# kallenordling/cesm_emulator

Hardware: NVIDIA B200
Metric: train samples/s (baseline cfg) (higher is better)
Workload: dtype fp16

## Files before the change

### cesm_emulator_b200/_lib.py

```python
from __future__ import annotations

import ctypes
from ctypes import POINTER, Structure, c_char_p, c_float, c_int32, c_int64, c_void_p
from pathlib import Path

_PKG = Path(__file__).resolve().parent
LIB_PATH = _PKG / "libcesm_b200.so"

CESM_MAX_TAPS = 16


class IgemmArgs(Structure):

    _fields_ = [
        ("a0", c_void_p), ("a1", c_void_p),
        ("c0", c_int32), ("c1", c_int32),
        ("n", c_int32), ("h", c_int32), ("w", c_int32),
        ("stride", c_int32),
        ("num_taps", c_int32),
        ("tap_dh", c_int32 * CESM_MAX_TAPS), ("tap_dw", c_int32 * CESM_MAX_TAPS),
        ("wt", c_void_p), ("cout", c_int32),
        ("oh", c_int32), ("ow", c_int32),
        ("out", c_void_p), ("ldo", c_int32),
        ("out_h", c_int32), ("out_w", c_int32),
        ("o_sh", c_int32), ("o_sw", c_int32), ("o_h0", c_int32), ("o_w0", c_int32),
        ("bias", c_void_p), ("residual", c_void_p), ("ldr", c_int32),
        ("gn_sums", c_void_p), ("gn_groups", c_int32), ("gn_frames", c_int32),
        ("ln_colsum", c_void_p), ("ln_eps", ctypes.c_float), ("reserved_", c_int32),
    ]


class WgradArgs(Structure):

    _fields_ = [
        ("x0", c_void_p), ("x1", c_void_p),
        ("c0", c_int32), ("c1", c_int32),
        ("n", c_int32), ("h", c_int32), ("w", c_int32),
        ("stride", c_int32),
        ("num_taps", c_int32),
        ("tap_dh", c_int32 * CESM_MAX_TAPS), ("tap_dw", c_int32 * CESM_MAX_TAPS),
        ("dy", c_void_p), ("cout", c_int32),
        ("oh", c_int32), ("ow", c_int32),
        ("y_h", c_int32), ("y_w", c_int32),
        ("y_sh", c_int32), ("y_sw", c_int32), ("y_h0", c_int32), ("y_w0", c_int32),
        ("dw", c_void_p),
        ("dw_so", ctypes.c_longlong), ("dw_si", ctypes.c_longlong),
        ("dw_tap_off", c_int32 * CESM_MAX_TAPS),
    ]


class PackDesc(Structure):

    _fields_ = [
        ("src", c_void_p), ("dst", c_void_p),
        ("O", c_int32), ("T", c_int32), ("I", c_int32), ("pad_", c_int32),
        ("so", ctypes.c_longlong), ("si", ctypes.c_longlong),
        ("tap_off", c_int32 * CESM_MAX_TAPS),
    ]


class FilmDesc(Structure):

    _fields_ = [("W", c_void_p), ("bias", c_void_p), ("dW", c_void_p), ("db", c_void_p), ("N", c_int32), ("n0", c_int32)]


class CesmError(RuntimeError):
    pass


_lib = None


def load() -> ctypes.CDLL:
    global _lib
    if _lib is not None:
        return _lib
    if not LIB_PATH.exists():
        raise CesmError(
            f"{LIB_PATH} not found: build it with `python -m cesm_emulator_b200.build` "
            "(there is no CPU or PyTorch fallback for the B200 kernels)")
    lib = ctypes.CDLL(str(LIB_PATH))
    lib.cesm_last_error.restype = c_char_p
    lib.cesm_version.restype = c_char_p
    lib.cesm_launch_count.restype = ctypes.c_longlong
    lib.cesm_linattn_ws_floats.restype = ctypes.c_size_t
    lib.cesm_linattn_ws_floats.argtypes = [ctypes.c_int, ctypes.c_int]
    lib.cesm_adamw_partials.restype = ctypes.c_int
    lib.cesm_tattn_long_max_frames.restype = ctypes.c_int
    lib.cesm_set_prezeroed_scratch.restype = None
    lib.cesm_set_prezeroed_scratch.argtypes = [ctypes.c_int]
    _declare(lib)
    _lib = lib
    return lib


_P, _I, _L, _F = c_void_p, ctypes.c_int, ctypes.c_longlong, c_float
_SIGNATURES: dict[str, list] = {
    "cesm_igemm": [POINTER(IgemmArgs), _P],
    "cesm_wgrad": [POINTER(WgradArgs), _P],
    "cesm_pack_weight": [_P, _P, _I, _I, _I, _L, _L, POINTER(c_int32), _P],
    "cesm_pack_weights_batched": [_P, _I, _P],
    "cesm_unpack_wgrads_batched": [_P, _I, _P],
    "cesm_unpack_wgrad": [_P, _P, _I, _I, _I, _L, _L, POINTER(c_int32), _I, _P],
    "cesm_adamw_step": [_P, _P, _P, _P, _L, _P, _P, _F, _F, _F, _F, _P],
    "cesm_adamw_ema_step": [_P, _P, _P, _P, _P, _L, _P, _P, _F, _F, _F, _F, ctypes.c_double, _L, _P],
    "cesm_colsum": [_P, _P, _L, _I, _I, _P],
    "cesm_gn_stats": [_P, _P, _I, _L, _I, _I, _P],
    "cesm_gn_apply_fwd": [_P, _P, _P, _P, _P, _P, _P, _I, _L, _I, _I, _F, _P],
    "cesm_gn_bwd": [_P, _P, _P, _P, _P, _P, _P, _P, _P, _P, _P, _P, _I, _L, _I, _I, _F, _I, _P],
    "cesm_ln_fwd": [_P, _P, _P, _L, _I, _F, _P],
    "cesm_ln_bwd": [_P, _P, _P, _P, _P, _P, _L, _I, _F, _I, _P],
    "cesm_tattn_fwd": [_P, _P, _P, _P, _P, _P, _I, _I, _I, _I, _I, _F, _P],
    "cesm_tattn_bwd": [_P, _P, _P, _P, _P, _P, _P, _P, _P, _I, _I, _I, _I, _I, _F, _P],
    "cesm_tattn_proj_fwd": [_P, _P, _P, _P, _P, _P, _I, _I, _I, _I, _I, _I, _F, _P],
    "cesm_tattn_long_fwd": [_P, _P, _P, _P, _P, _P, _I, _I, _I, _I, _I, _F, _P],
    "cesm_tattn_long_bwd": [_P, _P, _P, _P, _P, _P, _P, _P, _P, _I, _I, _I, _I, _I, _F, _P],
    "cesm_mattn_fwd": [_P, _P, _P, _I, _I, _I, _I, _F, _P],
    "cesm_mattn_bwd": [_P, _P, _P, _P, _P, _P, _I, _I, _I, _I, _F, _P],
    "cesm_linattn_fwd": [_P, _P, _P, _I, _I, _I, _I, _F, _P],
    "cesm_linattn_bwd": [_P, _P, _P, _P, _P, _I, _I, _I, _I, _F, _P],
    "cesm_film_fwd": [_P, _P, _P, _I, _I, _I, _I, _P],
    "cesm_film_bwd": [_P, _P, _P, _I, _I, _P, _I, _I, _I, _P],
    "cesm_gather_windows": [_P, _P, _P, _P, _P, _I, _I, _I, _I, _I, _I, _I, _I, _P],
    "cesm_qkv_bwd": [_P, _P, _P, _P, _P, _L, _L, _I, _I, _P],
    "cesm_input_patches": [_P, _P, _I, _I, _P, _I, _I, _I, _I, _I, _I, _P],
    "cesm_input_weight_pack": [_P, _P, _P, _I, _I, _I, _P],
    "cesm_input_conv_fwd": [_P, _P, _I, _I, _P, _P, _P, _I, _I, _I, _I, _I, _I, _P],
    "cesm_input_conv_wgrad": [_P, _P, _I, _I, _P, _P, _P, _I, _I, _I, _I, _I, _I, _P],
    "cesm_out_conv_fwd": [_P, _P, _P, _P, _I, _I, _I, _L, _I, _P],
    "cesm_out_conv_bwd": [_P, _P, _P, _P, _P, _P, _I, _I, _I, _L, _I, _P],
    "cesm_sinusoidal": [_P, _P, _I, _I, _P],
    "cesm_small_linear_fwd": [_P, _P, _P, _P, _I, _I, _I, _I, _P],
    "cesm_small_linear_bwd": [_P, _P, _P, _P, _P, _P, _I, _I, _I, _I, _I, _P],
    "cesm_q_sample": [_P, _P, _P, _P, _P, _P, _I, _L, _P],
    "cesm_mse_fwd": [_P, _P, _P, _P, _L, _P],
    "cesm_scale_by_scalar": [_P, _P, _F, _P, _L, _P],
    "cesm_p_sample": [_P, _P, _P, _P, _P, _P, _P, _P, _P, _I, _L, _P],
    "cesm_ddim_step": [_P, _P, _P, _P, _P, _P, _P, _P, _I, _I, _L, _P],
    "cesm_dpm_step": [_P, _P, _P, _P, _P, _P, _P, _P, _I, _I, _L, _P],
}


def _declare(lib: ctypes.CDLL) -> None:
    for name, argtypes in _SIGNATURES.items():
        fn = getattr(lib, name)
        fn.argtypes = argtypes
        fn.restype = ctypes.c_int


def exported_symbols() -> list[str]:
    return ["cesm_last_error", "cesm_version", "cesm_launch_count", "cesm_linattn_ws_floats", "cesm_adamw_partials",
            "cesm_set_prezeroed_scratch", "cesm_tattn_long_max_frames",
            *sorted(_SIGNATURES)]


def launch_count() -> int:
    return int(load().cesm_launch_count())


def check(rc: int, what: str) -> None:
    if rc != 0:
        msg = load().cesm_last_error().decode("utf-8", "replace")
        raise CesmError(f"{what} failed (status {rc}): {msg}")


class KernelProfiler:

    def __init__(self):
        self.records = []

    def summary(self):
        import torch
        torch.cuda.synchronize()
        out = {}
        for name, meta, e0, e1 in self.records:
            key = name if not meta or "kind" not in meta else f"{name}/{meta['kind']}"
            d = out.setdefault(key, {"calls": 0, "ms": 0.0, "flops": 0.0, "bytes": 0.0})
            d["calls"] += 1
            d["ms"] += e0.elapsed_time(e1)
            if meta:
                d["flops"] += meta.get("flops", 0.0)
                d["bytes"] += meta.get("bytes", 0.0)
        return out


PROFILER = None
NVTX = bool(int(__import__("os").environ.get("CESM_NVTX", "0")))


def _nvtx_call(lib, name, args, meta):
    from torch.cuda import nvtx
    nvtx.range_push(name if not meta or "kind" not in meta else f"{name}/{meta['kind']}")
    try:
        check(getattr(lib, name)(*args), name)
    finally:
        nvtx.range_pop()


def call(name: str, *args, _meta=None) -> None:
    lib = load()
    prof = PROFILER
    if prof is None:
        if NVTX:
            _nvtx_call(lib, name, args, _meta)
            return
        check(getattr(lib, name)(*args), name)
        return
    import torch
    e0, e1 = torch.cuda.Event(enable_timing=True), torch.cuda.Event(enable_timing=True)
    e0.record()
    check(getattr(lib, name)(*args), name)
    e1.record()
    prof.records.append((name, _meta, e0, e1))
```

### cesm_emulator_b200/csrc/linattn.cu

```cuda
#include "api_common.h"
#include "common.cuh"

namespace cesm {

static constexpr int LD = 32;
static constexpr int SPITCH = 40;

__device__ __forceinline__ void ldmatrix_x4_trans(uint32_t (&r)[4], uint32_t addr) {
    asm volatile("ldmatrix.sync.aligned.m8n8.x4.trans.shared.b16 {%0, %1, %2, %3}, [%4];"
                 : "=r"(r[0]), "=r"(r[1]), "=r"(r[2]), "=r"(r[3])
                 : "r"(addr));
}
__device__ __forceinline__ void mma_16816(float (&c)[4], const uint32_t (&a)[4], uint32_t b0, uint32_t b1) {
    asm volatile(
        "mma.sync.aligned.m16n8k16.row.col.f32.f16.f16.f32 {%0, %1, %2, %3}, {%4, %5, %6, %7}, {%8, %9}, "
        "{%0, %1, %2, %3};"
        : "+f"(c[0]), "+f"(c[1]), "+f"(c[2]), "+f"(c[3])
        : "r"(a[0]), "r"(a[1]), "r"(a[2]), "r"(a[3]), "r"(b0), "r"(b1));
}
__device__ __forceinline__ uint32_t enc_ordered(float f) {
    const uint32_t b = __float_as_uint(f);
    return (b & 0x80000000u) ? ~b : (b | 0x80000000u);
}
__device__ __forceinline__ float dec_ordered(uint32_t u) {
    return __uint_as_float((u & 0x80000000u) ? (u & 0x7fffffffu) : ~u);
}
__device__ __forceinline__ void unpack8(const uint4& u, float (&f)[8]) {
    float2 a = unpack_h2(u.x), b = unpack_h2(u.y), c = unpack_h2(u.z), d = unpack_h2(u.w);
    f[0] = a.x; f[1] = a.y; f[2] = b.x; f[3] = b.y; f[4] = c.x; f[5] = c.y; f[6] = d.x; f[7] = d.y;
}
__device__ __forceinline__ uint4 pack8(const float (&f)[8]) {
    uint4 u;
    u.x = pack_h2(f[0], f[1]); u.y = pack_h2(f[2], f[3]);
    u.z = pack_h2(f[4], f[5]); u.w = pack_h2(f[6], f[7]);
    return u;
}
__device__ __forceinline__ float quad_max(float v) {
    v = fmaxf(v, __shfl_xor_sync(0xffffffffu, v, 1));
    return fmaxf(v, __shfl_xor_sync(0xffffffffu, v, 2));
}
__device__ __forceinline__ float quad_sum(float v) {
    v += __shfl_xor_sync(0xffffffffu, v, 1);
    return v + __shfl_xor_sync(0xffffffffu, v, 2);
}

__device__ __forceinline__ void cp_async16(uint32_t dst, const void* src) {
    asm volatile("cp.async.cg.shared.global [%0], [%1], 16;" ::"r"(dst), "l"(src) : "memory");
}
__device__ __forceinline__ void cp_async_commit() { asm volatile("cp.async.commit_group;" ::: "memory"); }
template <int N>
__device__ __forceinline__ void cp_async_wait() {
    asm volatile("cp.async.wait_group %0;" ::"n"(N) : "memory");
}
static constexpr int kTileBytes = 16 * SPITCH * 2;

struct LaWs {
    uint32_t* kmax;
    float* z;
    float* ctx;
};
__device__ __forceinline__ LaWs la_ws(float* ws, int ni, int HD, int H) {
    float* base = ws + (size_t)ni * (2 * HD + (size_t)H * LD * LD);
    return {reinterpret_cast<uint32_t*>(base), base + HD, base + 2 * HD};
}

__global__ void __launch_bounds__(256)
la_colmax_kernel(const h16* __restrict__ qkv, float* __restrict__ ws, int n, int H, int rows_per_block) {
    pdl_trigger();
    pdl_wait();
    const int HD = H * LD, cpr = HD / 8;
    const int ni = blockIdx.y;
    const int chunk = threadIdx.x % cpr, rl = threadIdx.x / cpr, nrl = blockDim.x / cpr;
    const int p0 = blockIdx.x * rows_per_block, p1 = min(n, p0 + rows_per_block);
    float m[8];
#pragma unroll
    for (int i = 0; i < 8; ++i) m[i] = -INFINITY;
    if (rl < nrl) {
        const h16* base = qkv + ((size_t)ni * n) * (3 * HD) + HD + chunk * 8;
        for (int p = p0 + rl; p < p1; p += nrl) {
            float f[8];
            unpack8(__ldg(reinterpret_cast<const uint4*>(base + (size_t)p * 3 * HD)), f);
#pragma unroll
            for (int i = 0; i < 8; ++i) m[i] = fmaxf(m[i], f[i]);
        }
    }
    __shared__ float red[256][9];
#pragma unroll
    for (int i = 0; i < 8; ++i) red[threadIdx.x][i] = m[i];
    __syncthreads();
    if ((int)threadIdx.x < HD) {
        const int c = threadIdx.x, ch = c / 8, i = c % 8;
        float v = -INFINITY;
        for (int r = 0; r < nrl; ++r) v = fmaxf(v, red[r * cpr + ch][i]);
        if (v > -INFINITY) atomicMax(la_ws(ws, ni, HD, H).kmax + c, enc_ordered(v));
    }
}

static constexpr int CTX_STAGES = 3;
template <int MODE>
__global__ void __launch_bounds__(256)
la_context_kernel(const h16* __restrict__ qkv, const h16* __restrict__ dout,
                  float* __restrict__ ws, float* __restrict__ acc_out , int n, int H,
                  int chunk, float scale) {
    pdl_trigger();
    pdl_wait();
    extern __shared__ __align__(16) uint8_t la_smem[];
    const int HD = H * LD, ld = 3 * HD;
    const int ni = blockIdx.y, w = threadIdx.x >> 5, lane = threadIdx.x & 31;
    const int r = lane >> 2, c = lane & 3;
    constexpr int kWarpTiles = 2 * CTX_STAGES + (MODE == 1 ? 1 : 0);
    uint8_t* wbase = la_smem + (size_t)w * kWarpTiles * kTileBytes;
    h16* sA = reinterpret_cast<h16*>(wbase + 2 * CTX_STAGES * kTileBytes);
    const uint32_t sA_addr = smem_u32(sA);
    const uint32_t ring_addr = smem_u32(wbase);
    const LaWs W = la_ws(ws, ni, HD, H);

    float cmf[2][2], zf[2][2];
#pragma unroll
    for (int mt = 0; mt < 2; ++mt)
#pragma unroll
        for (int hh = 0; hh < 2; ++hh) {
            cmf[mt][hh] = (MODE == 0) ? dec_ordered(W.kmax[w * LD + 16 * mt + r + 8 * hh]) * kLog2e : 0.f;
            zf[mt][hh] = 0.f;
        }
    float acc[2][4][4];
#pragma unroll
    for (int a = 0; a < 2; ++a)
#pragma unroll
        for (int b = 0; b < 4; ++b)
#pragma unroll
            for (int k = 0; k < 4; ++k) acc[a][b][k] = 0.f;

    const size_t img_row0 = (size_t)ni * n;
    const h16* a_base = qkv + img_row0 * ld + (MODE == 0 ? HD : 0) + w * LD + c * 8;
    const h16* b_base = (MODE == 0) ? qkv + img_row0 * ld + 2 * HD + w * LD + c * 8
                                              : dout + img_row0 * HD + w * LD + c * 8;
    const int b_ld = (MODE == 0) ? ld : HD;
    const int p0 = blockIdx.x * chunk, p1 = min(n, p0 + chunk);

    const int mi = lane >> 3, rr = lane & 7;
    uint32_t a_off[2], b_off[2];
#pragma unroll
    for (int mt = 0; mt < 2; ++mt) a_off[mt] = (((mi >> 1) * 8 + rr) * SPITCH + 16 * mt + (mi & 1) * 8) * 2;
#pragma unroll
    for (int jp = 0; jp < 2; ++jp) b_off[jp] = (((mi & 1) * 8 + rr) * SPITCH + 8 * (jp * 2 + (mi >> 1))) * 2;

    auto issue_loads = [&](int step) {
        const int pp = p0 + 16 * step;
        const uint32_t st = ring_addr + (step % CTX_STAGES) * 2 * kTileBytes;
        if (pp < p1) {
#pragma unroll
            for (int h2 = 0; h2 < 2; ++h2) {
                const int row = min(pp + r + 8 * h2, p1 - 1);
                const uint32_t off = ((r + 8 * h2) * SPITCH + c * 8) * 2;
                cp_async16(st + off, a_base + (size_t)row * ld);
                cp_async16(st + kTileBytes + off, b_base + (size_t)row * b_ld);
            }
        }
        cp_async_commit();
    };
    const int nsteps = (p1 - p0 + 15) / 16;
#pragma unroll
    for (int s0 = 0; s0 < CTX_STAGES - 1; ++s0) issue_loads(s0);
    for (int step = 0; step < nsteps; ++step) {
        const int p = p0 + 16 * step;
        issue_loads(step + CTX_STAGES - 1);
        cp_async_wait<CTX_STAGES - 1>();
        __syncwarp();
        const uint32_t st = ring_addr + (step % CTX_STAGES) * 2 * kTileBytes;
        const uint32_t sB_addr = st + kTileBytes;
        uint32_t af[2][4], bf[2][4];
        if (MODE == 0) {
            ldmatrix_x4_trans(af[0], st + a_off[0]);
            ldmatrix_x4_trans(af[1], st + a_off[1]);
            const bool full = p + 16 <= p1;
#pragma unroll
            for (int mt = 0; mt < 2; ++mt)
#pragma unroll
                for (int i = 0; i < 4; ++i) {
                    const float2 x = unpack_h2(af[mt][i]);
                    float e0 = exp_sub(x.x, cmf[mt][i & 1]), e1 = exp_sub(x.y, cmf[mt][i & 1]);
                    if (!full) {
                        const int px = p + 2 * c + 8 * (i >> 1);
                        e0 = px < p1 ? e0 : 0.f;
                        e1 = px + 1 < p1 ? e1 : 0.f;
                    }
                    zf[mt][i & 1] += e0 + e1;
                    af[mt][i] = pack_h2(e0, e1);
                }
        } else {
            uint4 ua[2];
#pragma unroll
            for (int h2 = 0; h2 < 2; ++h2) {
                const uint32_t off = ((r + 8 * h2) * SPITCH + c * 8) * 2;
                asm volatile("ld.shared.v4.b32 {%0, %1, %2, %3}, [%4];"
                             : "=r"(ua[h2].x), "=r"(ua[h2].y), "=r"(ua[h2].z), "=r"(ua[h2].w)
                             : "r"(st + off));
            }
#pragma unroll
            for (int h2 = 0; h2 < 2; ++h2) {
                const bool valid = (p + r + 8 * h2) < p1;
                float f[8];
                unpack8(ua[h2], f);
                float m = f[0];
#pragma unroll
                for (int i = 1; i < 8; ++i) m = fmaxf(m, f[i]);
                m = quad_max(m) * kLog2e;
                float sum = 0.f;
#pragma unroll
                for (int i = 0; i < 8; ++i) {
                    f[i] = exp_sub(f[i], m);
                    sum += f[i];
                }
                sum = quad_sum(sum);
                const float inv = valid ? scale / sum : 0.f;
#pragma unroll
                for (int i = 0; i < 8; ++i) f[i] *= inv;
                *reinterpret_cast<uint4*>(sA + (r + 8 * h2) * SPITCH + c * 8) = pack8(f);
            }
            __syncwarp();
            ldmatrix_x4_trans(af[0], sA_addr + a_off[0]);
            ldmatrix_x4_trans(af[1], sA_addr + a_off[1]);
        }
        ldmatrix_x4_trans(bf[0], sB_addr + b_off[0]);
        ldmatrix_x4_trans(bf[1], sB_addr + b_off[1]);
        __syncwarp();
#pragma unroll
        for (int mt = 0; mt < 2; ++mt)
#pragma unroll
            for (int j = 0; j < 4; ++j) mma_16816(acc[mt][j], af[mt], bf[j >> 1][(j & 1) * 2], bf[j >> 1][(j & 1) * 2 + 1]);
    }

    float* dst = (MODE == 0 ? W.ctx : acc_out + (size_t)ni * H * LD * LD) + (size_t)w * LD * LD;
    const int g = lane >> 2, t = lane & 3;
#pragma unroll
    for (int mt = 0; mt < 2; ++mt)
#pragma unroll
        for (int j = 0; j < 4; ++j) {
            const int d0 = 16 * mt + g, e0 = 8 * j + 2 * t;
            atomicAdd(dst + d0 * LD + e0, acc[mt][j][0]);
            atomicAdd(dst + d0 * LD + e0 + 1, acc[mt][j][1]);
            atomicAdd(dst + (d0 + 8) * LD + e0, acc[mt][j][2]);
            atomicAdd(dst + (d0 + 8) * LD + e0 + 1, acc[mt][j][3]);
        }
    if (MODE == 0) {
#pragma unroll
        for (int mt = 0; mt < 2; ++mt)
#pragma unroll
            for (int hh = 0; hh < 2; ++hh) {
                const float z = quad_sum(zf[mt][hh]);
                if (c == 0) atomicAdd(W.z + w * LD + 16 * mt + r + 8 * hh, z);
            }
    }
}

__global__ void la_finalize_kernel(float* __restrict__ ws, int H, int NI) {
    pdl_trigger();
    pdl_wait();
    const int HD = H * LD;
    const int idx = blockIdx.x * blockDim.x + threadIdx.x;
    const int per = H * LD * LD;
    if (idx >= NI * per) return;
    const int ni = idx / per, x = idx % per;
    const LaWs W = la_ws(ws, ni, HD, H);
    W.ctx[x] = W.ctx[x] / W.z[x / LD];
}

__global__ void la_delta_kernel(float* __restrict__ ws, const float* __restrict__ dctx, float* __restrict__ delta,
                                int H, int NI) {
    pdl_trigger();
    pdl_wait();
    const int HD = H * LD;
    const int idx = blockIdx.x * blockDim.x + threadIdx.x;
    if (idx >= NI * HD) return;
    const int ni = idx / HD, hd = idx % HD;
    const LaWs W = la_ws(ws, ni, HD, H);
    const float* dc = dctx + ((size_t)ni * HD + hd) * LD;
    float s = 0.f;
#pragma unroll
    for (int e = 0; e < LD; ++e) s = fmaf(W.ctx[hd * LD + e], dc[e], s);
    delta[idx] = s;
}

__device__ __forceinline__ int phi32(int L) { return ((L >> 1) & 3) * 8 + (L >> 3) * 2 + (L & 1); }

template <bool TRANS>
__device__ __forceinline__ void load_bfrag32(const float* __restrict__ M, int g, int t, uint32_t (&b)[2][4][2]) {
#pragma unroll
    for (int ks = 0; ks < 2; ++ks)
#pragma unroll
        for (int j = 0; j < 4; ++j) {
            const int nn = phi32(8 * j + g);
#pragma unroll
            for (int hi = 0; hi < 2; ++hi) {
                const int k0 = phi32(16 * ks + 8 * hi + 2 * t), k1 = k0 + 1;
                b[ks][j][hi] = TRANS ? pack_h2(M[nn * LD + k0], M[nn * LD + k1])
                                     : pack_h2(M[k0 * LD + nn], M[k1 * LD + nn]);
            }
        }
}
__device__ __forceinline__ void rows_to_afrag(const uint4& lo, const uint4& hi, uint32_t (&a)[2][4]) {
    a[0][0] = lo.x; a[0][1] = hi.x; a[0][2] = lo.y; a[0][3] = hi.y;
    a[1][0] = lo.z; a[1][1] = hi.z; a[1][2] = lo.w; a[1][3] = hi.w;
}
__device__ __forceinline__ void frag_gemm(const uint32_t (&a)[2][4], const uint32_t (&b)[2][4][2], float (&c)[4][4]) {
#pragma unroll
    for (int j = 0; j < 4; ++j) {
        c[j][0] = c[j][1] = c[j][2] = c[j][3] = 0.f;
#pragma unroll
        for (int ks = 0; ks < 2; ++ks) mma_16816(c[j], a[ks], b[ks][j][0], b[ks][j][1]);
    }
}
__device__ __forceinline__ void c_to_rows(const float (&c)[4][4], float (&o)[2][8]) {
#pragma unroll
    for (int j = 0; j < 4; ++j) {
        o[0][2 * j] = c[j][0]; o[0][2 * j + 1] = c[j][1];
        o[1][2 * j] = c[j][2]; o[1][2 * j + 1] = c[j][3];
    }
}
__device__ __forceinline__ void row_softmax(float (&f)[8]) {
    float m = f[0];
#pragma unroll
    for (int i = 1; i < 8; ++i) m = fmaxf(m, f[i]);
    m = quad_max(m) * kLog2e;
    float s = 0.f;
#pragma unroll
    for (int i = 0; i < 8; ++i) {
        f[i] = exp_sub(f[i], m);
        s += f[i];
    }
    const float inv = 1.f / quad_sum(s);
#pragma unroll
    for (int i = 0; i < 8; ++i) f[i] *= inv;
}

static constexpr int APPLY_MT = 2;
static constexpr int RING_STAGES = 3;
__device__ __forceinline__ uint4 lds16(uint32_t addr) {
    uint4 u;
    asm volatile("ld.shared.v4.b32 {%0, %1, %2, %3}, [%4];" : "=r"(u.x), "=r"(u.y), "=r"(u.z), "=r"(u.w) : "r"(addr));
    return u;
}
__global__ void __launch_bounds__(256, 3)
la_apply_kernel(const h16* __restrict__ qkv, float* __restrict__ ws, h16* __restrict__ out, int n,
                int H, int chunk, float scale) {
    pdl_trigger();
    pdl_wait();
    extern __shared__ __align__(16) uint8_t la_smem[];
    const int HD = H * LD, ld = 3 * HD;
    const int ni = blockIdx.y, w = threadIdx.x >> 5, lane = threadIdx.x & 31;
    const int r = lane >> 2, c = lane & 3;
    const LaWs W = la_ws(ws, ni, HD, H);
    uint32_t bctx[2][4][2];
    load_bfrag32<false>(W.ctx + (size_t)w * LD * LD, r, c, bctx);
    const size_t row0 = (size_t)ni * n;
    const int p1 = min(n, (int)(blockIdx.x + 1) * chunk);
    const h16* qbase = qkv + row0 * ld + w * LD + c * 8;
    h16* obase = out + row0 * HD + w * LD + c * 8;
    const uint32_t ring = smem_u32(la_smem) + threadIdx.x * 16u;
    constexpr uint32_t kVec = 256 * 16, kStage = APPLY_MT * 2 * kVec;
    auto issue_loads = [&](int pp, int stage) {
        if (pp < p1) {
#pragma unroll
            for (int mt = 0; mt < APPLY_MT; ++mt)
#pragma unroll
                for (int h2 = 0; h2 < 2; ++h2) {
                    const int row = min(pp + 16 * mt + r + 8 * h2, p1 - 1);
                    cp_async16(ring + stage * kStage + (mt * 2 + h2) * kVec, qbase + (size_t)row * ld);
                }
        }
        cp_async_commit();
    };
    const int pstart = blockIdx.x * chunk;
#pragma unroll
    for (int s0 = 0; s0 < RING_STAGES - 1; ++s0) issue_loads(pstart + s0 * 16 * APPLY_MT, s0);
    int stage = 0;
    for (int p = pstart; p < p1; p += 16 * APPLY_MT) {
        {
            int ns = stage + RING_STAGES - 1;
            if (ns >= RING_STAGES) ns -= RING_STAGES;
            issue_loads(p + (RING_STAGES - 1) * 16 * APPLY_MT, ns);
        }
        cp_async_wait<RING_STAGES - 1>();
        uint4 cq[APPLY_MT][2];
#pragma unroll
        for (int mt = 0; mt < APPLY_MT; ++mt)
#pragma unroll
            for (int h2 = 0; h2 < 2; ++h2) cq[mt][h2] = lds16(ring + stage * kStage + (mt * 2 + h2) * kVec);
        if (++stage == RING_STAGES) stage = 0;
#pragma unroll
        for (int mt = 0; mt < APPLY_MT; ++mt) {
            uint4 pk[2];
#pragma unroll
            for (int h2 = 0; h2 < 2; ++h2) {
                float f[8];
                unpack8(cq[mt][h2], f);
                row_softmax(f);
#pragma unroll
                for (int i = 0; i < 8; ++i) f[i] *= scale;
                pk[h2] = pack8(f);
            }
            uint32_t a[2][4];
            rows_to_afrag(pk[0], pk[1], a);
            float cfr[4][4], o[2][8];
            frag_gemm(a, bctx, cfr);
            c_to_rows(cfr, o);
#pragma unroll
            for (int h2 = 0; h2 < 2; ++h2) {
                const int row = p + 16 * mt + r + 8 * h2;
                if (row < p1) *reinterpret_cast<uint4*>(obase + (size_t)row * HD) = pack8(o[h2]);
            }
        }
    }
}

__global__ void __launch_bounds__(256, 2)
la_bwd_apply_kernel(const h16* __restrict__ qkv, const h16* __restrict__ dout,
                    float* __restrict__ ws, const float* __restrict__ dctx, const float* __restrict__ delta,
                    h16* __restrict__ dqkv, int n, int H, int chunk, float scale) {
    pdl_trigger();
    pdl_wait();
    extern __shared__ __align__(16) uint8_t la_smem[];
    const int HD = H * LD, ld = 3 * HD;
    const int ni = blockIdx.y, w = threadIdx.x >> 5, lane = threadIdx.x & 31;
    const int r = lane >> 2, c = lane & 3;
    const LaWs W = la_ws(ws, ni, HD, H);
    const float* dcx = dctx + ((size_t)ni * H + w) * LD * LD;
    uint32_t b_ctxT[2][4][2], b_dctxT[2][4][2], b_dctx[2][4][2];
    load_bfrag32<true>(W.ctx + (size_t)w * LD * LD, r, c, b_ctxT);
    load_bfrag32<true>(dcx, r, c, b_dctxT);
    load_bfrag32<false>(dcx, r, c, b_dctx);
    __shared__ __align__(16) float s_kml[8 * LD], s_del[8 * LD];
    {
        const int col = threadIdx.x;
        s_kml[col] = (dec_ordered(W.kmax[col]) + __logf(W.z[col])) * kLog2e;
        s_del[col] = delta[(size_t)ni * HD + col];
    }
    __syncthreads();
    const float* kml = s_kml + w * LD + c * 8;
    const float* del = s_del + w * LD + c * 8;
    const size_t row0 = (size_t)ni * n;
    const int p1 = min(n, (int)(blockIdx.x + 1) * chunk);
    const h16* xbase = qkv + row0 * ld + w * LD + c * 8;
    const h16* dbase = dout + row0 * HD + w * LD + c * 8;
    h16* gbase = dqkv + row0 * ld + w * LD + c * 8;
    const uint32_t ring = smem_u32(la_smem) + threadIdx.x * 16u;
    constexpr uint32_t kVec = 256 * 16, kStage = 8 * kVec;
    auto issue_loads = [&](int pp, int stage) {
        if (pp < p1) {
#pragma unroll
            for (int h2 = 0; h2 < 2; ++h2) {
                const int row = min(pp + r + 8 * h2, p1 - 1);
                const h16* xg = xbase + (size_t)row * ld;
                const uint32_t st = ring + stage * kStage + h2 * 4 * kVec;
                cp_async16(st, dbase + (size_t)row * HD);
                cp_async16(st + kVec, xg);
                cp_async16(st + 2 * kVec, xg + HD);
                cp_async16(st + 3 * kVec, xg + 2 * HD);
            }
        }
        cp_async_commit();
    };
    const int pstart = blockIdx.x * chunk;
#pragma unroll
    for (int s0 = 0; s0 < RING_STAGES - 1; ++s0) issue_loads(pstart + s0 * 16, s0);
    int stage = 0;
    for (int p = pstart; p < p1; p += 16) {
        {
            int ns = stage + RING_STAGES - 1;
            if (ns >= RING_STAGES) ns -= RING_STAGES;
            issue_loads(p + (RING_STAGES - 1) * 16, ns);
        }
        cp_async_wait<RING_STAGES - 1>();
        float sm[2][8];
        uint4 ud[2], uv[2], uk[2];
#pragma unroll
        for (int h2 = 0; h2 < 2; ++h2) {
            const uint32_t st = ring + stage * kStage + h2 * 4 * kVec;
            ud[h2] = lds16(st);
            unpack8(lds16(st + kVec), sm[h2]);
            uk[h2] = lds16(st + 2 * kVec);
            uv[h2] = lds16(st + 3 * kVec);
        }
        if (++stage == RING_STAGES) stage = 0;
#pragma unroll
        for (int h2 = 0; h2 < 2; ++h2) row_softmax(sm[h2]);
        uint32_t a[2][4];
        float cfr[4][4], o[2][8];
        rows_to_afrag(ud[0], ud[1], a);
        frag_gemm(a, b_ctxT, cfr);
        c_to_rows(cfr, o);
#pragma unroll
        for (int h2 = 0; h2 < 2; ++h2) {
            float dot = 0.f;
#pragma unroll
            for (int i = 0; i < 8; ++i) dot = fmaf(sm[h2][i], o[h2][i], dot);
            dot = quad_sum(dot);
#pragma unroll
            for (int i = 0; i < 8; ++i) o[h2][i] = sm[h2][i] * scale * (o[h2][i] - dot);
            const int row = p + r + 8 * h2;
            if (row < p1) *reinterpret_cast<uint4*>(gbase + (size_t)row * ld) = pack8(o[h2]);
        }
        rows_to_afrag(uv[0], uv[1], a);
        frag_gemm(a, b_dctxT, cfr);
        c_to_rows(cfr, o);
        uint4 ukh[2];
#pragma unroll
        for (int h2 = 0; h2 < 2; ++h2) {
            float kh[8], km[8], dl[8];
            unpack8(uk[h2], kh);
            *reinterpret_cast<float4*>(km) = *reinterpret_cast<const float4*>(kml);
            *reinterpret_cast<float4*>(km + 4) = *reinterpret_cast<const float4*>(kml + 4);
            *reinterpret_cast<float4*>(dl) = *reinterpret_cast<const float4*>(del);
            *reinterpret_cast<float4*>(dl + 4) = *reinterpret_cast<const float4*>(del + 4);
#pragma unroll
            for (int i = 0; i < 8; ++i) {
                kh[i] = exp_sub(kh[i], km[i]);
                o[h2][i] = kh[i] * (o[h2][i] - dl[i]);
            }
            ukh[h2] = pack8(kh);
            const int row = p + r + 8 * h2;
            if (row < p1) *reinterpret_cast<uint4*>(gbase + (size_t)row * ld + HD) = pack8(o[h2]);
        }
        rows_to_afrag(ukh[0], ukh[1], a);
        frag_gemm(a, b_dctx, cfr);
        c_to_rows(cfr, o);
#pragma unroll
        for (int h2 = 0; h2 < 2; ++h2) {
            const int row = p + r + 8 * h2;
            if (row < p1) *reinterpret_cast<uint4*>(gbase + (size_t)row * ld + 2 * HD) = pack8(o[h2]);
        }
    }
}

}

using namespace cesm;

static int la_chunk(int n, int NI) {
    int chunk = 2048;
    while (chunk > 128 && (long long)NI * ((n + chunk - 1) / chunk) < 148 * 4) chunk >>= 1;
    return chunk;
}

static size_t la_context_smem(int H, int mode) {
    static bool cfg = false;
    if (!cfg) {
        cudaFuncSetAttribute(la_context_kernel<0>, cudaFuncAttributeMaxDynamicSharedMemorySize, 8 * 2 * CTX_STAGES * kTileBytes);
        cudaFuncSetAttribute(la_context_kernel<1>, cudaFuncAttributeMaxDynamicSharedMemorySize, 8 * (2 * CTX_STAGES + 1) * kTileBytes);
        cfg = true;
    }
    return (size_t)H * (2 * CTX_STAGES + (mode == 1 ? 1 : 0)) * kTileBytes;
}

extern "C" size_t cesm_linattn_ws_floats(int NI, int H) { return (size_t)NI * (2 * H * LD + (size_t)H * LD * LD); }

extern "C" int cesm_linattn_fwd(const void* qkv, float* ws, void* out, int NI, int n, int H, int dim_head, float scale,
                                void* stream) {
    CESM_REQUIRE(dim_head == LD, "linear attention kernel needs dim_head == 32 (got %d)", dim_head);
    CESM_REQUIRE(H >= 1 && H <= 8, "linear attention kernel supports 1..8 heads (got %d)", H);
    cudaStream_t st = as_stream(stream);
    const int HD = H * LD;
    CESM_ZERO_SCRATCH(ws, sizeof(float) * cesm_linattn_ws_floats(NI, H), st);
    const int chunk = la_chunk(n, NI);
    dim3 grid(ceil_div(n, chunk), NI);
    launch_pdl(la_colmax_kernel, grid, 256, 0, st, (const h16*)qkv, ws, n, H, chunk);
    CESM_CHECK_LAUNCH();
    const size_t sh = la_context_smem(H, 0);
    launch_pdl(la_context_kernel<0>, grid, 32 * H, sh, st, (const h16*)qkv, nullptr, ws, nullptr, n, H, chunk, scale);
    CESM_CHECK_LAUNCH();
    launch_pdl(la_finalize_kernel, ceil_div(NI * H * LD * LD, 256), 256, 0, st, ws, H, NI);
    CESM_CHECK_LAUNCH();
    const size_t sh_apply = (size_t)RING_STAGES * APPLY_MT * 2 * 256 * 16;
    launch_pdl(la_apply_kernel, grid, 32 * H, sh_apply, st, (const h16*)qkv, ws, (h16*)out, n, H, chunk,
                                                    scale);
    CESM_CHECK_LAUNCH();
    (void)HD;
    return CESM_OK;
}

extern "C" int cesm_linattn_bwd(const void* qkv, float* ws, const void* dout, float* scratch, void* dqkv, int NI, int n,
                                int H, int dim_head, float scale, void* stream) {
    CESM_REQUIRE(dim_head == LD, "linear attention kernel needs dim_head == 32 (got %d)", dim_head);
    CESM_REQUIRE(H >= 1 && H <= 8, "linear attention kernel supports 1..8 heads (got %d)", H);
    cudaStream_t st = as_stream(stream);
    float* dctx = scratch;
    float* delta = scratch + (size_t)NI * H * LD * LD;
    CESM_ZERO_SCRATCH(dctx, sizeof(float) * NI * H * LD * LD, st);
    const int chunk = la_chunk(n, NI);
    dim3 grid(ceil_div(n, chunk), NI);
    const size_t sh = la_context_smem(H, 1);
    launch_pdl(la_context_kernel<1>, grid, 32 * H, sh, st, (const h16*)qkv, (const h16*)dout, ws, dctx, n, H,
                                                   chunk, scale);
    CESM_CHECK_LAUNCH();
    launch_pdl(la_delta_kernel, ceil_div(NI * H * LD, 128), 128, 0, st, ws, dctx, delta, H, NI);
    CESM_CHECK_LAUNCH();
    const size_t sh_bwd = (size_t)RING_STAGES * 8 * 256 * 16;
    static bool bwd_cfg = false;
    if (!bwd_cfg) {
        CESM_CHECK_CUDA(cudaFuncSetAttribute(la_bwd_apply_kernel, cudaFuncAttributeMaxDynamicSharedMemorySize, (int)sh_bwd));
        bwd_cfg = true;
    }
    launch_pdl(la_bwd_apply_kernel, grid, 32 * H, sh_bwd, st, (const h16*)qkv, (const h16*)dout, ws, dctx, delta,
                                                 (h16*)dqkv, n, H, chunk, scale);
    CESM_CHECK_LAUNCH();
    return CESM_OK;
}
```

### cesm_emulator_b200/kernels.py

```python
from __future__ import annotations

import ctypes
from typing import Optional, Sequence, Tuple

import torch

from . import _lib
from ._lib import IgemmArgs

H16 = torch.float16


def _stream() -> ctypes.c_void_p:
    return ctypes.c_void_p(torch.cuda.current_stream().cuda_stream)


def _ptr(t: Optional[torch.Tensor]) -> Optional[int]:
    return None if t is None else t.data_ptr()


def _req_cuda(*ts: Optional[torch.Tensor]) -> None:
    for t in ts:
        if t is not None and not t.is_cuda:
            raise _lib.CesmError("cesm_emulator_b200 kernels need CUDA tensors (no CPU fallback)")
        if t is not None and not t.is_contiguous():
            raise _lib.CesmError("cesm_emulator_b200 kernels need contiguous tensors")


def _bytes_meta(*ts, kind=None):
    if _lib.PROFILER is None:
        return None
    m = {"bytes": float(sum(t.numel() * t.element_size() for t in ts if t is not None))}
    if kind:
        m["kind"] = kind
    return m


TAPS_3x3 = [(dh, dw) for dh in (-1, 0, 1) for dw in (-1, 0, 1)]
TAPS_1x1 = [(0, 0)]


class ZeroArena:

    def __init__(self, device, floats: int = 4 << 20):
        self.buf = torch.zeros(floats, dtype=torch.float32, device=device)
        self.off = 0
        self.high = 0

    def begin(self) -> None:
        global _ARENA
        if self.high:
            self.buf[:self.high].zero_()
        self.off = 0
        _ARENA = self
        _lib.load().cesm_set_prezeroed_scratch(1)

    def end(self) -> None:
        global _ARENA
        _ARENA = None
        _lib.load().cesm_set_prezeroed_scratch(0)

    def take(self, shape) -> torch.Tensor:
        n = 1
        for d in shape:
            n *= int(d)
        start = self.off
        self.off = start + (n + 63) // 64 * 64
        if self.off > self.buf.numel():
            self.off = start
            return torch.zeros(tuple(shape), dtype=torch.float32, device=self.buf.device)
        self.high = max(self.high, self.off)
        return self.buf[start:start + n].view(*shape)


_ARENA: Optional[ZeroArena] = None


def zero_scratch(shape, device) -> torch.Tensor:
    if _ARENA is not None:
        return _ARENA.take(tuple(shape))
    return torch.empty(tuple(shape), dtype=torch.float32, device=device)


def igemm(a0: torch.Tensor, wt: torch.Tensor, *, taps: Sequence[Tuple[int, int]] = TAPS_1x1,
          a1: Optional[torch.Tensor] = None, stride: int = 1,
          out: Optional[torch.Tensor] = None, out_hw: Optional[Tuple[int, int]] = None,
          out_place: Tuple[int, int, int, int] = (1, 1, 0, 0),
          bias: Optional[torch.Tensor] = None, residual: Optional[torch.Tensor] = None,
          gn_sums: Optional[torch.Tensor] = None, gn_frames: int = 1,
          ln_fold: Optional[Tuple[torch.Tensor, float]] = None):
    _req_cuda(a0, a1, wt, out, bias, residual)
    assert a0.dtype == H16 and wt.dtype == H16 and a0.dim() == 4
    n, h, w, c0 = a0.shape
    c1 = 0 if a1 is None else a1.shape[-1]
    cout = wt.shape[0]
    assert wt.shape[1] == len(taps) * (c0 + c1), (wt.shape, len(taps), c0, c1)
    oh, ow = out_hw if out_hw is not None else (h // stride, w // stride)
    o_sh, o_sw, o_h0, o_w0 = out_place
    if out is None:
        assert out_place == (1, 1, 0, 0)
        out = torch.empty((n, oh, ow, cout), dtype=H16, device=a0.device)
    assert out.dtype == H16, out.dtype
    args = IgemmArgs()
    args.a0, args.a1, args.c0, args.c1 = _ptr(a0), _ptr(a1), c0, c1
    args.n, args.h, args.w, args.stride = n, h, w, stride
    args.num_taps = len(taps)
    for i, (dh, dw) in enumerate(taps):
        args.tap_dh[i], args.tap_dw[i] = dh, dw
    args.wt, args.cout = _ptr(wt), cout
    args.oh, args.ow = oh, ow
    args.out, args.ldo = _ptr(out), out.shape[-1]
    args.out_h, args.out_w = out.shape[1], out.shape[2]
    args.o_sh, args.o_sw, args.o_h0, args.o_w0 = o_sh, o_sw, o_h0, o_w0
    args.bias = _ptr(bias)
    args.residual = _ptr(residual)
    args.ldr = 0 if residual is None else residual.shape[-1]
    if gn_sums is not None:
        assert gn_sums.dtype == torch.float32 and gn_sums.dim() == 3 and gn_sums.shape[0] * gn_frames == n
        args.gn_sums, args.gn_groups, args.gn_frames = _ptr(gn_sums), gn_sums.shape[1], gn_frames
    if ln_fold is not None:
        cs, eps = ln_fold
        assert residual is not None and residual.data_ptr() == a0.data_ptr() and c0 == 64 and cout == 64 and a1 is None
        assert cs.dtype == torch.float32 and cs.numel() == cout and cs.is_cuda
        args.ln_colsum, args.ln_eps = _ptr(cs), float(eps)
    if bias is not None:
        assert bias.dtype == torch.float32 and bias.numel() == cout
    if residual is not None:
        assert residual.dtype == H16 and residual.shape[:3] == out.shape[:3]
    meta = None
    if _lib.PROFILER is not None:
        rows = n * oh * ow
        ktot = len(taps) * (c0 + c1)
        meta = {"kind": f"{len(taps)}tap", "flops": 2.0 * rows * cout * ktot,
                "bytes": 2.0 * (rows * (c0 + c1) * stride * stride + rows * cout + cout * ktot)}
    _lib.call("cesm_igemm", ctypes.byref(args), _stream(), _meta=meta)
    return out


def wgrad(x0: torch.Tensor, dy: torch.Tensor, *, taps: Sequence[Tuple[int, int]] = TAPS_1x1,
          x1: Optional[torch.Tensor] = None, stride: int = 1, grid_hw: Optional[Tuple[int, int]] = None,
          dy_place: Tuple[int, int, int, int] = (1, 1, 0, 0), into: Optional[torch.Tensor] = None,
          layout: Optional[Tuple[int, int, Sequence[int]]] = None) -> torch.Tensor:
    _req_cuda(x0, x1, dy)
    assert x0.dtype == H16 and dy.dtype == H16 and x0.dim() == 4 and dy.dim() == 4
    n, h, w, c0 = x0.shape
    c1 = 0 if x1 is None else x1.shape[-1]
    cout = dy.shape[-1]
    oh, ow = grid_hw if grid_hw is not None else (h // stride, w // stride)
    a = _lib.WgradArgs()
    if into is not None:
        assert layout is not None and into.dtype == torch.float32 and into.is_contiguous()
        dw_ = into
        a.dw_so, a.dw_si = int(layout[0]), int(layout[1])
        for i, o in enumerate(layout[2]):
            a.dw_tap_off[i] = int(o)
    else:
        dw_ = torch.empty((cout, len(taps), c0 + c1), dtype=torch.float32, device=x0.device)
    a.x0, a.x1, a.c0, a.c1 = _ptr(x0), _ptr(x1), c0, c1
    a.n, a.h, a.w, a.stride = n, h, w, stride
    a.num_taps = len(taps)
    for i, (dh, dw) in enumerate(taps):
        a.tap_dh[i], a.tap_dw[i] = dh, dw
    a.dy, a.cout, a.oh, a.ow = _ptr(dy), cout, oh, ow
    a.y_h, a.y_w = dy.shape[1], dy.shape[2]
    a.y_sh, a.y_sw, a.y_h0, a.y_w0 = dy_place
    a.dw = _ptr(dw_)
    meta = None
    if _lib.PROFILER is not None:
        rows = n * oh * ow
        meta = {"kind": f"{len(taps)}tap", "flops": 2.0 * rows * cout * len(taps) * (c0 + c1),
                "bytes": 2.0 * rows * (c0 + c1 + cout) + 4.0 * cout * len(taps) * (c0 + c1)}
    _lib.call("cesm_wgrad", ctypes.byref(a), _stream(), _meta=meta)
    return dw_


def qkv_bwd(dy: torch.Tensor, x: torch.Tensor, wt: torch.Tensor, dw_into: Optional[torch.Tensor] = None):
    _req_cuda(dy, x, wt, dw_into)
    assert dy.dtype == H16 and x.dtype == H16 and wt.dtype == H16 and dy.is_contiguous() and x.is_contiguous()
    cout, cin = dy.shape[-1], x.shape[-1]
    rows = x.numel() // cin
    assert dy.numel() // cout == rows and tuple(wt.shape) == (cin, cout) and wt.is_contiguous()
    dx = torch.empty_like(x)
    if dw_into is None:
        dw = torch.zeros((cout, cin), dtype=torch.float32, device=x.device)
    else:
        assert dw_into.dtype == torch.float32 and dw_into.is_contiguous() and dw_into.numel() == cout * cin
        dw = dw_into
    meta = None
    if _lib.PROFILER is not None:
        meta = {"kind": "qkv", "flops": 4.0 * rows * cout * cin, "bytes": 2.0 * rows * (cout + 2 * cin)}
    _lib.call("cesm_qkv_bwd", _ptr(dy), _ptr(x), _ptr(wt), _ptr(dx), _ptr(dw), cin, rows, cin, cout, _stream(), _meta=meta)
    return dx, dw


def _tap_array(offs: Sequence[int]):
    arr = (ctypes.c_int32 * _lib.CESM_MAX_TAPS)()
    for i, o in enumerate(offs):
        arr[i] = int(o)
    return arr


def pack_weight(src: torch.Tensor, O: int, T: int, I: int, so: int, si: int, tap_off: Sequence[int],
                out: Optional[torch.Tensor] = None) -> torch.Tensor:
    _req_cuda(src)
    assert src.dtype == torch.float32
    if out is None:
        out = torch.empty((O, T * I), dtype=H16, device=src.device)
    _lib.call("cesm_pack_weight", _ptr(src), _ptr(out), O, T, I, so, si, _tap_array(tap_off), _stream())
    return out


def unpack_wgrad(src: torch.Tensor, dst: torch.Tensor, O: int, T: int, I: int, so: int, si: int,
                 tap_off: Sequence[int], accumulate: bool = False) -> torch.Tensor:
    _req_cuda(src, dst)
    assert src.dtype == torch.float32 and dst.dtype == torch.float32
    _lib.call("cesm_unpack_wgrad", _ptr(src), _ptr(dst), O, T, I, so, si, _tap_array(tap_off), int(accumulate), _stream())
    return dst


OPT_STATE_FLOATS = 16
OPT_STEP, OPT_NORM, OPT_SCALE, OPT_TRACKER, OPT_FOUND_INF, OPT_SKIPPED, OPT_LR, OPT_WD, OPT_INTERVAL = range(9)


def adamw_step(p: torch.Tensor, g: torch.Tensor, m: torch.Tensor, v: torch.Tensor, partials: torch.Tensor,
               state: torch.Tensor, beta1: float, beta2: float, eps: float, max_norm: Optional[float]) -> None:
    _req_cuda(p, g, m, v, partials, state)
    for t in (p, g, m, v, partials, state):
        assert t.dtype == torch.float32 and t.is_contiguous()
    assert p.numel() == g.numel() == m.numel() == v.numel() and state.numel() >= OPT_STATE_FLOATS
    assert partials.numel() >= _lib.load().cesm_adamw_partials()
    _lib.call("cesm_adamw_step", _ptr(p), _ptr(g), _ptr(m), _ptr(v), p.numel(), _ptr(partials), _ptr(state),
              float(beta1), float(beta2), float(eps), float(max_norm) if max_norm is not None else 0.0, _stream(),
              _meta={"bytes": 28.0 * p.numel()})


def adamw_ema_step(p: torch.Tensor, g: torch.Tensor, m: torch.Tensor, v: torch.Tensor, ema: torch.Tensor,
                   partials: torch.Tensor, state: torch.Tensor, beta1: float, beta2: float, eps: float,
                   max_norm: Optional[float], ema_decay: float, ema_start: int) -> None:
    _req_cuda(p, g, m, v, ema, partials, state)
    for t in (p, g, m, v, ema, partials, state):
        assert t.dtype == torch.float32 and t.is_contiguous()
    assert p.numel() == g.numel() == m.numel() == v.numel() == ema.numel() and state.numel() >= OPT_STATE_FLOATS
    assert partials.numel() >= _lib.load().cesm_adamw_partials()
    _lib.call("cesm_adamw_ema_step", _ptr(p), _ptr(g), _ptr(m), _ptr(v), _ptr(ema), p.numel(), _ptr(partials),
              _ptr(state), float(beta1), float(beta2), float(eps), float(max_norm) if max_norm is not None else 0.0,
              float(ema_decay), int(ema_start), _stream(), _meta={"bytes": 36.0 * p.numel()})


def colsum(x: torch.Tensor, into: Optional[torch.Tensor] = None) -> torch.Tensor:
    _req_cuda(x, into)
    C = x.shape[-1]
    out = torch.empty(C, dtype=torch.float32, device=x.device) if into is None else into
    _lib.call("cesm_colsum", _ptr(x), _ptr(out), x.numel() // C, C, int(into is not None), _stream())
    return out


def gn_stats(x: torch.Tensor, B: int, G: int) -> torch.Tensor:
    _req_cuda(x)
    C = x.shape[-1]
    P = x.numel() // (B * C)
    sums = torch.empty((B, G, 2), dtype=torch.float32, device=x.device)
    _lib.call("cesm_gn_stats", _ptr(x), _ptr(sums), B, P, C, G, _stream(), _meta=_bytes_meta(x))
    return sums


def gn_apply_fwd(x, sums, gamma, beta, film, residual, B: int, G: int, eps: float) -> torch.Tensor:
    _req_cuda(x, sums, gamma, beta, film, residual)
    C = x.shape[-1]
    P = x.numel() // (B * C)
    out = torch.empty_like(x)
    _lib.call("cesm_gn_apply_fwd", _ptr(x), _ptr(sums), _ptr(gamma), _ptr(beta), _ptr(film), _ptr(residual), _ptr(out),
              B, P, C, G, eps, _stream(), _meta=_bytes_meta(x, residual, out))
    return out


def gn_bwd(x, dout, sums, gamma, beta, film, B: int, G: int, eps: float, conv_bias_grad: bool = False,
           into=None):
    _req_cuda(x, dout, sums, gamma, beta, film)
    C = x.shape[-1]
    P = x.numel() // (B * C)
    dev = x.device
    csum = zero_scratch((B, C, 3), dev)
    dx = torch.empty_like(x)
    if into is not None:
        dgamma, dbeta, dcb = into
    else:
        dgamma = torch.empty(C, dtype=torch.float32, device=dev)
        dbeta = torch.empty(C, dtype=torch.float32, device=dev)
        dcb = torch.empty(C, dtype=torch.float32, device=dev) if conv_bias_grad else None
    dfilm = torch.empty((B, 2 * C), dtype=torch.float32, device=dev) if film is not None else None
    _lib.call("cesm_gn_bwd", _ptr(x), _ptr(dout), _ptr(sums), _ptr(gamma), _ptr(beta), _ptr(film), _ptr(csum), _ptr(dx),
              _ptr(dgamma), _ptr(dbeta), _ptr(dfilm), _ptr(dcb), B, P, C, G, eps, int(into is not None), _stream(),
              _meta=_bytes_meta(x, dout, x, dout, dx))
    if conv_bias_grad:
        return dx, dgamma, dbeta, dfilm, dcb
    return dx, dgamma, dbeta, dfilm


def ln_fwd(x: torch.Tensor, gamma: torch.Tensor, eps: float) -> torch.Tensor:
    _req_cuda(x, gamma)
    C = x.shape[-1]
    out = torch.empty_like(x)
    _lib.call("cesm_ln_fwd", _ptr(x), _ptr(gamma), _ptr(out), x.numel() // C, C, eps, _stream(),
              _meta=_bytes_meta(x, out))
    return out


def ln_bwd(x, gamma, dy, dres, eps: float, into: Optional[torch.Tensor] = None):
    _req_cuda(x, gamma, dy, dres, into)
    C = x.shape[-1]
    dx = torch.empty_like(x)
    dgamma = torch.empty(C, dtype=torch.float32, device=x.device) if into is None else into
    _lib.call("cesm_ln_bwd", _ptr(x), _ptr(gamma), _ptr(dy), _ptr(dres), _ptr(dx), _ptr(dgamma), x.numel() // C, C, eps,
              int(into is not None), _stream(), _meta=_bytes_meta(x, dy, dres, dx))
    return dx, dgamma


LONG_WINDOW_MAX = 128


def _bias_to_diag(bias: torch.Tensor) -> torch.Tensor:
    return torch.cat([bias[:, 1:, 0].flip(1), bias[:, 0, :]], dim=1).contiguous()


def _diag_to_bias_grad(ddiag: torch.Tensor, F: int) -> torch.Tensor:
    H = ddiag.shape[0]
    g = torch.zeros((H, F, F), dtype=ddiag.dtype, device=ddiag.device)
    g[:, 0, :] = ddiag[:, F - 1:]
    g[:, 1:, 0] = ddiag[:, :F - 1].flip(1)
    return g


def tattn_fwd(qkv, bias, cs, sn, B: int, F: int, HW: int, H: int, D: int, scale: float):
    _req_cuda(qkv, bias, cs, sn)
    rows = B * F * HW
    out = torch.empty((rows, H * D), dtype=H16, device=qkv.device)
    if 4 < F <= LONG_WINDOW_MAX:
        lse = torch.empty((rows, H), dtype=torch.float32, device=qkv.device)
        _lib.call("cesm_tattn_long_fwd", _ptr(qkv), _ptr(_bias_to_diag(bias)), _ptr(cs), _ptr(sn), _ptr(out), _ptr(lse),
                  B, F, HW, H, D, scale, _stream(),
                  _meta={"kind": f"F{F}", "bytes": float(qkv.numel() * 2 + out.numel() * 2),
                         "flops": 4.0 * rows * H * F * D * 2})
        return out, lse
    lse = torch.empty((rows, H), dtype=torch.float32, device=qkv.device) if F > 4 else None
    _lib.call("cesm_tattn_fwd", _ptr(qkv), _ptr(bias), _ptr(cs), _ptr(sn), _ptr(out), _ptr(lse), B, F, HW, H, D, scale,
              _stream(), _meta=_bytes_meta(qkv, out))
    return out, lse


def tattn_bwd(qkv, bias, cs, sn, out, lse, dout, B: int, F: int, HW: int, H: int, D: int, scale: float):
    _req_cuda(qkv, bias, cs, sn, out, lse, dout)
    dqkv = torch.empty_like(qkv)
    if 4 < F <= LONG_WINDOW_MAX:
        ddiag = zero_scratch((H, 2 * F - 1), qkv.device)
        _lib.call("cesm_tattn_long_bwd", _ptr(qkv), _ptr(_bias_to_diag(bias)), _ptr(cs), _ptr(sn), _ptr(out), _ptr(lse),
                  _ptr(dout), _ptr(dqkv), _ptr(ddiag), B, F, HW, H, D, scale, _stream(),
                  _meta={"kind": f"F{F}", "bytes": float(qkv.numel() * 4 + dout.numel() * 4),
                         "flops": 14.0 * B * F * HW * H * F * D * 2})
        return dqkv, _diag_to_bias_grad(ddiag, F)
    dbias = zero_scratch((H, F, F), qkv.device)
    _lib.call("cesm_tattn_bwd", _ptr(qkv), _ptr(bias), _ptr(cs), _ptr(sn), _ptr(out), _ptr(lse), _ptr(dout), _ptr(dqkv),
              _ptr(dbias), B, F, HW, H, D, scale, _stream(), _meta=_bytes_meta(qkv, dout, dqkv))
    return dqkv, dbias


def tattn_proj_ok(C: int, F: int, HW: int, H: int, D: int) -> bool:
    return C == 64 and 1 <= F <= 3 and HW % 16 == 0 and H == 8 and D == 32


def tattn_proj_fwd(xn, wqkv_packed, bias, cs, sn, B: int, F: int, HW: int, H: int, D: int, scale: float):
    _req_cuda(xn, wqkv_packed, bias, cs, sn)
    assert xn.dtype == H16 and wqkv_packed.dtype == H16 and tuple(wqkv_packed.shape) == (3 * H * D, 64)
    rows = B * F * HW
    out = torch.empty((rows, H * D), dtype=H16, device=xn.device)
    _lib.call("cesm_tattn_proj_fwd", _ptr(xn), _ptr(wqkv_packed), _ptr(bias), _ptr(cs), _ptr(sn), _ptr(out), B, F, HW, H, D,
              64, scale, _stream(),
              _meta={"kind": "fused", "flops": 2.0 * rows * 64 * 3 * H * D, "bytes": float(rows * (64 + H * D) * 2)})
    return out


def mattn_fwd(qkv, NI: int, n: int, H: int, D: int, scale: float):
    _req_cuda(qkv)
    assert qkv.dtype == H16 and qkv.shape == (NI * n, 3 * H * D), (tuple(qkv.shape), NI, n, H, D)
    out = torch.empty((NI * n, H * D), dtype=H16, device=qkv.device)
    lse = torch.empty((NI * n, H), dtype=torch.float32, device=qkv.device)
    _lib.call("cesm_mattn_fwd", _ptr(qkv), _ptr(out), _ptr(lse), NI, n, H, D, scale, _stream(),
              _meta={"kind": "fwd", "flops": 4.0 * NI * H * n * n * D, "bytes": float(qkv.numel() * 2 + out.numel() * 2)})
    return out, lse


def mattn_bwd(qkv, out, lse, dout, NI: int, n: int, H: int, D: int, scale: float):
    _req_cuda(qkv, out, lse, dout)
    assert qkv.dtype == H16 and out.dtype == H16 and dout.dtype == H16 and lse.dtype == torch.float32
    assert qkv.shape == (NI * n, 3 * H * D) and out.shape == dout.shape == (NI * n, H * D) and lse.numel() == NI * n * H
    dqkv = torch.empty_like(qkv)
    delta = torch.empty((NI * n, H), dtype=torch.float32, device=qkv.device)
    _lib.call("cesm_mattn_bwd", _ptr(qkv), _ptr(out), _ptr(lse), _ptr(dout), _ptr(dqkv), _ptr(delta), NI, n, H, D, scale,
              _stream(), _meta={"kind": "bwd", "flops": 14.0 * NI * H * n * n * D,
                                "bytes": float(qkv.numel() * 4 + out.numel() * 2 + dout.numel() * 2)})
    return dqkv


def linattn_fwd(qkv, NI: int, n: int, H: int, D: int, scale: float):
    _req_cuda(qkv)
    dev = qkv.device
    ws = zero_scratch((_lib.load().cesm_linattn_ws_floats(NI, H),), dev)
    out = torch.empty((NI * n, H * D), dtype=H16, device=dev)
    _lib.call("cesm_linattn_fwd", _ptr(qkv), _ptr(ws), _ptr(out), NI, n, H, D, scale, _stream(),
              _meta=_bytes_meta(qkv, out))
    return out, ws


def linattn_bwd(qkv, ws, dout, NI: int, n: int, H: int, D: int, scale: float):
    _req_cuda(qkv, ws, dout)
    scratch = zero_scratch((NI * H * D * D + NI * H * D,), qkv.device)
    dqkv = torch.empty_like(qkv)
    _lib.call("cesm_linattn_bwd", _ptr(qkv), _ptr(ws), _ptr(dout), _ptr(scratch), _ptr(dqkv), NI, n, H, D, scale,
              _stream(), _meta=_bytes_meta(qkv, dout, dqkv))
    return dqkv


def gather_windows(cond, tgt, plan, cond_out, x0_out) -> None:
    _req_cuda(cond, tgt, plan, cond_out, x0_out)
    assert cond.dtype == tgt.dtype == cond_out.dtype == x0_out.dtype == torch.float32 and plan.dtype == torch.int32
    assert cond.is_contiguous() and tgt.is_contiguous() and cond_out.is_contiguous() and x0_out.is_contiguous()
    T, M, H, W = cond.shape
    B, _, K, h, w = cond_out.shape
    assert plan.shape == (B, 6) and plan.is_contiguous() and x0_out.shape == (B, 1, h, w) and tgt.shape == cond.shape
    _lib.call("cesm_gather_windows", _ptr(cond), _ptr(tgt), _ptr(plan), _ptr(cond_out), _ptr(x0_out), B, T, M, H, W, K,
              h, w, _stream())


INPUT_KPAD = 256


def input_patches(in0, in1, B: int, F: int, H: int, W: int, ks: int) -> torch.Tensor:
    _req_cuda(in0, in1)
    f0, f1 = in0.numel() // (B * H * W), in1.numel() // (B * H * W)
    out = torch.empty((B * F, H, W, INPUT_KPAD), dtype=H16, device=in0.device)
    _lib.call("cesm_input_patches", _ptr(in0), _ptr(in1), f0, f1, _ptr(out), B, F, H, W, ks, INPUT_KPAD, _stream(),
              _meta=_bytes_meta(out))
    return out


def input_weight_pack(w, bias, out: Optional[torch.Tensor] = None) -> torch.Tensor:
    _req_cuda(w, bias)
    cout, ks = w.shape[0], w.shape[-1]
    if out is None:
        out = torch.empty((cout, INPUT_KPAD), dtype=H16, device=w.device)
    _lib.call("cesm_input_weight_pack", _ptr(w), _ptr(bias), _ptr(out), cout, ks, INPUT_KPAD, _stream())
    return out


def input_conv_fwd(in0, in1, w, bias, B: int, F: int, H: int, W: int, ks: int):
    _req_cuda(in0, in1, w, bias)
    cout = w.shape[0]
    f0, f1 = in0.numel() // (B * H * W), in1.numel() // (B * H * W)
    out = torch.empty((B * F, H, W, cout), dtype=H16, device=in0.device)
    _lib.call("cesm_input_conv_fwd", _ptr(in0), _ptr(in1), f0, f1, _ptr(w), _ptr(bias), _ptr(out), B, F, H, W, ks, cout,
              _stream())
    return out


def input_conv_wgrad(in0, in1, dy, B: int, F: int, H: int, W: int, ks: int):
    _req_cuda(in0, in1, dy)
    cout = dy.shape[-1]
    f0, f1 = in0.numel() // (B * H * W), in1.numel() // (B * H * W)
    dw = torch.empty((cout, 2, 1, ks, ks), dtype=torch.float32, device=dy.device)
    db = torch.empty(cout, dtype=torch.float32, device=dy.device)
    _lib.call("cesm_input_conv_wgrad", _ptr(in0), _ptr(in1), f0, f1, _ptr(dy), _ptr(dw), _ptr(db), B, F, H, W, ks, cout,
              _stream())
    return dw, db


def out_conv_fwd(a, w, bias, B: int, F: int, H: int, W: int, mid: Optional[int] = None):
    _req_cuda(a, w, bias)
    mid = F // 2 if mid is None else mid
    eps = torch.empty((B, 1, H, W), dtype=torch.float32, device=a.device)
    _lib.call("cesm_out_conv_fwd", _ptr(a), _ptr(w), _ptr(bias), _ptr(eps), B, F, mid, H * W, a.shape[-1], _stream())
    return eps


def out_conv_bwd(a, w, deps, B: int, F: int, H: int, W: int, mid: Optional[int] = None):
    _req_cuda(a, w, deps)
    mid = F // 2 if mid is None else mid
    da = torch.empty_like(a)
    dw = torch.empty_like(w)
    db = torch.empty(1, dtype=torch.float32, device=a.device)
    _lib.call("cesm_out_conv_bwd", _ptr(a), _ptr(w), _ptr(deps), _ptr(da), _ptr(dw), _ptr(db), B, F, mid, H * W,
              a.shape[-1], _stream())
    return da, dw, db


def sinusoidal(t: torch.Tensor, dim: int) -> torch.Tensor:
    _req_cuda(t)
    assert t.dtype == torch.int64
    out = torch.empty((t.numel(), dim), dtype=torch.float32, device=t.device)
    _lib.call("cesm_sinusoidal", _ptr(t), _ptr(out), t.numel(), dim, _stream())
    return out


def small_linear_fwd(x, W, bias, act_silu_in: bool):
    _req_cuda(x, W, bias)
    B, K = x.shape
    N = W.shape[0]
    y = torch.empty((B, N), dtype=torch.float32, device=x.device)
    _lib.call("cesm_small_linear_fwd", _ptr(x), _ptr(W), _ptr(bias), _ptr(y), B, K, N, int(act_silu_in), _stream())
    return y


def small_linear_bwd(x, W, dy, act_silu_in: bool, need_dx: bool, into=None):
    _req_cuda(x, W, dy)
    B, K = x.shape
    N = W.shape[0]
    if into is not None:
        dW, db = into
    else:
        dW = torch.empty_like(W)
        db = torch.empty(N, dtype=torch.float32, device=x.device)
    dx = torch.empty_like(x) if need_dx else None
    _lib.call("cesm_small_linear_bwd", _ptr(x), _ptr(W), _ptr(dy), _ptr(dx), _ptr(dW), _ptr(db), B, K, N,
              int(act_silu_in), int(into is not None), _stream())
    return dx, dW, db


def film_table(Ws, bs, dWs=None, dbs=None) -> torch.Tensor:
    n = len(Ws)
    arr = (_lib.FilmDesc * n)()
    n0 = 0
    for i, d in enumerate(arr):
        d.W, d.bias = Ws[i].data_ptr(), bs[i].data_ptr()
        d.dW = dWs[i].data_ptr() if dWs is not None else 0
        d.db = dbs[i].data_ptr() if dbs is not None else 0
        d.N, d.n0 = Ws[i].shape[0], n0
        n0 += Ws[i].shape[0]
    return torch.frombuffer(bytearray(bytes(arr)), dtype=torch.uint8).to(Ws[0].device)


def film_fwd(x: torch.Tensor, table: torch.Tensor, Ns) -> list:
    _req_cuda(x, table)
    B, K = x.shape
    n_total = int(sum(Ns))
    y = torch.empty(B * n_total, dtype=torch.float32, device=x.device)
    _lib.call("cesm_film_fwd", _ptr(x), _ptr(table), _ptr(y), len(Ns), n_total, B, K, _stream())
    outs, n0 = [], 0
    for N in Ns:
        outs.append(y[B * n0:B * (n0 + N)].view(B, N))
        n0 += N
    return outs


def film_bwd(x: torch.Tensor, table: torch.Tensor, dy_packed: torch.Tensor, Ns, need_dx: bool, accumulate: bool):
    _req_cuda(x, table, dy_packed)
    B, K = x.shape
    n_total = int(sum(Ns))
    assert dy_packed.numel() == B * n_total and dy_packed.dtype == torch.float32 and dy_packed.is_contiguous()
    dx = zero_scratch(x.shape, x.device) if need_dx else None
    _lib.call("cesm_film_bwd", _ptr(x), _ptr(table), _ptr(dy_packed), len(Ns), n_total, _ptr(dx), B, K, int(accumulate),
              _stream())
    return dx


def q_sample(x0, noise, t, sqrt_ac, sqrt_1mac):
    _req_cuda(x0, noise, t, sqrt_ac, sqrt_1mac)
    xt = torch.empty_like(x0)
    B = x0.shape[0]
    _lib.call("cesm_q_sample", _ptr(x0), _ptr(noise), _ptr(t), _ptr(sqrt_ac), _ptr(sqrt_1mac), _ptr(xt), B,
              x0.numel() // B, _stream())
    return xt


def mse_fwd(eps, noise):
    _req_cuda(eps, noise)
    diff = torch.empty_like(eps)
    loss = torch.empty((), dtype=torch.float32, device=eps.device)
    _lib.call("cesm_mse_fwd", _ptr(eps), _ptr(noise), _ptr(diff), _ptr(loss), eps.numel(), _stream())
    return loss, diff


def scale_by_scalar(x, gscale, factor: float):
    _req_cuda(x, gscale)
    out = torch.empty_like(x)
    _lib.call("cesm_scale_by_scalar", _ptr(x), _ptr(gscale), factor, _ptr(out), x.numel(), _stream())
    return out


def p_sample(xt, eps, z, t, betas, sqrt_1mac, sqrt_recip_a, post_var):
    _req_cuda(xt, eps, z, t, betas, sqrt_1mac, sqrt_recip_a, post_var)
    out = torch.empty_like(xt)
    B = xt.shape[0]
    _lib.call("cesm_p_sample", _ptr(xt), _ptr(eps), _ptr(z), _ptr(t), _ptr(betas), _ptr(sqrt_1mac), _ptr(sqrt_recip_a),
              _ptr(post_var), _ptr(out), B, xt.numel() // B, _stream())
    return out


def ddim_step(xt, eps, z, t, coef, T: int, out=None, next_t=None, t_out=None):
    _req_cuda(xt, eps, z, t, coef, out, next_t, t_out)
    assert coef.dtype == torch.float32 and coef.shape == (T, 3), (coef.dtype, tuple(coef.shape), T)
    assert t.dtype == torch.int64 and xt.dtype == eps.dtype == torch.float32 and eps.shape == xt.shape
    assert z is None or (z.dtype == torch.float32 and z.shape == xt.shape)
    assert (t_out is None) == (next_t is None), "next_t and t_out go together"
    assert next_t is None or (next_t.dtype == torch.int64 and next_t.shape == (T,) and t_out.dtype == torch.int64)
    out = torch.empty_like(xt) if out is None else out
    assert out.dtype == torch.float32 and out.shape == xt.shape
    B = xt.shape[0]
    _lib.call("cesm_ddim_step", _ptr(xt), _ptr(eps), _ptr(z), _ptr(t), _ptr(coef), _ptr(next_t), _ptr(t_out), _ptr(out),
              T, B, xt.numel() // B, _stream())
    return out


def dpm_step(xt, eps, hist, t, coef, T: int, out=None, next_t=None, t_out=None):
    _req_cuda(xt, eps, hist, t, coef, out, next_t, t_out)
    assert coef.dtype == torch.float32 and coef.shape == (T, 5), (coef.dtype, tuple(coef.shape), T)
    assert t.dtype == torch.int64 and xt.dtype == eps.dtype == torch.float32 and eps.shape == xt.shape
    assert hist.dtype == torch.float32 and hist.shape == xt.shape
    assert (t_out is None) == (next_t is None), "next_t and t_out go together"
    assert next_t is None or (next_t.dtype == torch.int64 and next_t.shape == (T,) and t_out.dtype == torch.int64)
    out = torch.empty_like(xt) if out is None else out
    assert out.dtype == torch.float32 and out.shape == xt.shape
    B = xt.shape[0]
    _lib.call("cesm_dpm_step", _ptr(xt), _ptr(eps), _ptr(hist), _ptr(t), _ptr(coef), _ptr(next_t), _ptr(t_out),
              _ptr(out), T, B, xt.numel() // B, _stream())
    return out
```

### cesm_emulator_b200/ops.py

```python
from __future__ import annotations

import weakref
from typing import Optional, Tuple

import torch

from . import _lib
from . import kernels as K

H16 = torch.float16

_PHASE_TAPS = {0: [(0, 1), (-1, 3)], 1: [(1, 0), (0, 2)]}


_OUTER_GRAD = [True]


class _Fn(torch.autograd.Function):
    @classmethod
    def apply(cls, *args, **kwargs):
        _OUTER_GRAD[0] = torch.is_grad_enabled()
        return super().apply(*args, **kwargs)


def _train(ctx) -> bool:
    return _OUTER_GRAD[0] and any(ctx.needs_input_grad)


def _c(t: Optional[torch.Tensor]) -> Optional[torch.Tensor]:
    return None if t is None else t.contiguous()


def _phase(ph: int, pw: int):
    taps, koff = [], []
    for dh, kh in _PHASE_TAPS[ph]:
        for dw, kw in _PHASE_TAPS[pw]:
            taps.append((dh, dw))
            koff.append(kh * 4 + kw)
    return taps, koff


_WEIGHT_EPOCH = [0]


def invalidate_weight_cache(*_args, **_kwargs) -> None:
    _WEIGHT_EPOCH[0] += 1


try:
    from torch.optim.optimizer import register_optimizer_step_post_hook as _reg_hook
    _reg_hook(invalidate_weight_cache)
except Exception:
    pass


class _PackEntry:
    __slots__ = ("wref", "src_off", "O", "T", "I", "so", "si", "taps", "out", "key", "serial")


_ENTRIES: list = []
_PLAN = {"n": -1, "ptrs": None, "descs": None}
_PREPACK_SERIAL = [0]


def _key(weight: torch.Tensor):
    return (weight.data_ptr(), weight._version, _WEIGHT_EPOCH[0])


class PackCache:

    def __init__(self):
        self._d = {}

    def get(self, weight: torch.Tensor, tag, spec, train: bool = False) -> torch.Tensor:
        ent = self._d.get(tag)
        if ent is None or ent.wref() is not weight:
            ent = _PackEntry()
            ent.wref = weakref.ref(weight)
            ent.src_off, ent.O, ent.T, ent.I, ent.so, ent.si, ent.taps = spec
            ent.out = torch.empty((ent.O, ent.T * ent.I), dtype=H16, device=weight.device)
            ent.key, ent.serial = None, -1
            self._d[tag] = ent
            _ENTRIES.append(ent)
        key = _key(weight)
        force = (train and weight.is_cuda and torch.cuda.is_current_stream_capturing()
                 and ent.serial != _PREPACK_SERIAL[0])
        if force or ent.key != key:
            src = weight.detach().reshape(-1)
            if ent.src_off:
                src = src[ent.src_off:]
            K.pack_weight(src, ent.O, ent.T, ent.I, ent.so, ent.si, ent.taps, out=ent.out)
            ent.key, ent.serial = key, _PREPACK_SERIAL[0]
        return ent.out

    def __deepcopy__(self, memo):
        return PackCache()


def prepack_all() -> int:
    live = [e for e in _ENTRIES if e.wref() is not None]
    if len(live) != len(_ENTRIES):
        _ENTRIES[:] = live
    if not live:
        return 0
    ptrs = tuple((e.wref().data_ptr(), e.out.data_ptr()) for e in live)
    if _PLAN["n"] != len(live) or _PLAN["ptrs"] != ptrs:
        arr = (_lib.PackDesc * len(live))()
        for d, e in zip(arr, live):
            d.src = e.wref().data_ptr() + 4 * e.src_off
            d.dst = e.out.data_ptr()
            d.O, d.T, d.I, d.so, d.si = e.O, e.T, e.I, e.so, e.si
            for i, o in enumerate(e.taps):
                d.tap_off[i] = int(o)
        host = torch.frombuffer(bytearray(bytes(arr)), dtype=torch.uint8)
        _PLAN.update(n=len(live), ptrs=ptrs, descs=host.to(live[0].out.device))
    _PREPACK_SERIAL[0] += 1
    _lib.call("cesm_pack_weights_batched", _PLAN["descs"].data_ptr(), len(live), K._stream())
    for e in live:
        e.key, e.serial = _key(e.wref()), _PREPACK_SERIAL[0]
    return len(live)


_FOLDS: list = []


def _fold_compute(ent, wqkv, wout, gamma) -> None:
    C, hidden = ent[1].shape[0], ent[4]
    wv = wqkv.detach().reshape(3 * hidden, C)[2 * hidden:].float()
    wo = wout.detach().reshape(C, hidden).float()
    w = wo @ wv
    ent[1].copy_(w)
    if gamma is not None:
        ent[6].copy_(w * gamma.detach().reshape(1, C).float())
        ent[7].copy_(ent[6].float().sum(dim=1))


def _fold_f1(meta, wqkv, wout, hidden: int, C: int, gamma=None):
    key = (_key(wqkv), _key(wout), None if gamma is None else _key(gamma))
    ent = meta.__dict__.get("fold_f1")
    if ent is None or ent[1].device != wqkv.device or (gamma is not None and ent[5] is None):
        dev = wqkv.device
        ent = [None, torch.empty((C, C), dtype=H16, device=dev), weakref.ref(wqkv), weakref.ref(wout), hidden,
               None if gamma is None else weakref.ref(gamma),
               None if gamma is None else torch.empty((C, C), dtype=H16, device=dev),
               None if gamma is None else torch.empty((C,), dtype=torch.float32, device=dev)]
        meta.__dict__["fold_f1"] = ent
        _FOLDS.append(ent)
    if ent[0] != key:
        _fold_compute(ent, wqkv, wout, gamma)
        ent[0] = key
    return ent[1] if gamma is None else (ent[6], ent[7])


def refresh_folds() -> None:
    live = [e for e in _FOLDS if e[2]() is not None and e[3]() is not None and (e[5] is None or e[5]() is not None)]
    _FOLDS[:] = live
    for e in live:
        wqkv, wout = e[2](), e[3]()
        gamma = None if e[5] is None else e[5]()
        key = (_key(wqkv), _key(wout), None if gamma is None else _key(gamma))
        if e[0] != key:
            _fold_compute(e, wqkv, wout, gamma)
            e[0] = key


_GRAD_SINK = [None]


def set_grad_sink(sink) -> None:
    _GRAD_SINK[0] = sink


def _direct(weight: torch.Tensor) -> bool:
    sink = _GRAD_SINK[0]
    return sink is not None and weight.grad is not None and sink.owns(weight)


def _direct_all(*params) -> bool:
    return all(p is not None and _direct(p) for p in params)


def _ready(*params) -> None:
    for p in params:
        _GRAD_SINK[0].ready(p)


_SIDE = [None]
_SIDE_KEEP: list = []


def set_side_stream(stream) -> None:
    _SIDE[0] = stream
    _SIDE_KEEP.clear()


def join_side_stream() -> None:
    side = _SIDE[0]
    if side is not None:
        torch.cuda.current_stream().wait_stream(side)
    _SIDE_KEEP.clear()


class _on_side:

    def __init__(self, *tensors):
        self.side = _SIDE[0] if _GRAD_SINK[0] is not None else None
        self.tensors = tensors
        self.ctx = None

    def __enter__(self):
        if self.side is not None:
            self.side.wait_stream(torch.cuda.current_stream())
            _SIDE_KEEP.append(self.tensors)
            self.ctx = torch.cuda.stream(self.side)
            self.ctx.__enter__()
        return self

    def __exit__(self, *exc):
        if self.ctx is not None:
            self.ctx.__exit__(*exc)
        return False


def _wgrad_into_param(weight, x0, x1, dy, taps, so, si, tap_off, last: bool = True,
                      into: Optional[torch.Tensor] = None, **kw):
    T = len(taps)
    if _direct(weight):
        sink = _GRAD_SINK[0]
        with _on_side(x0, x1, dy):
            if T == 1:
                K.wgrad(x0, dy, x1=x1, taps=taps, into=weight.grad, layout=(so, si, tap_off), **kw)
            else:
                cout = dy.shape[-1]
                ctot = x0.shape[-1] + (0 if x1 is None else x1.shape[-1])
                scratch = sink.scratch(weight, tuple(tap_off), (cout, T, ctot, so, si, list(tap_off)))
                K.wgrad(x0, dy, x1=x1, taps=taps, into=scratch, layout=(T * ctot, 1, [t * ctot for t in range(T)]), **kw)
        if last:
            sink.ready(weight)
        return None
    dwt = torch.zeros_like(weight) if into is None else into
    K.wgrad(x0, dy, x1=x1, taps=taps, into=dwt, layout=(so, si, tap_off), **kw)
    return dwt


def _sq_taps(ks: int):
    r = ks // 2
    return [(kh - r, kw - r) for kh in range(ks) for kw in range(ks)]


def _conv_fwd_weight(cache: PackCache, weight, cout: int, ctot: int, ks: int, train: bool):
    kk = ks * ks
    return cache.get(weight, "fwd", (0, cout, kk, ctot, ctot * kk, kk, list(range(kk))), train)


def _conv_dgrad_weights(cache: PackCache, weight, cout: int, c0: int, c1: int, ks: int, train: bool):
    if not train:
        return None, None
    kk, ctot = ks * ks, c0 + c1
    w0 = cache.get(weight, "dgrad0", (0, c0, kk, cout, kk, ctot * kk, list(range(kk))), train)
    w1 = (cache.get(weight, "dgrad1", (c0 * kk, c1, kk, cout, kk, ctot * kk, list(range(kk))), train)
          if c1 else None)
    return w0, w1


def _bias_grad(bias, dy):
    if bias is not None and _direct_all(bias):
        with _on_side(dy):
            K.colsum(dy, into=bias.grad)
        _ready(bias)
        return None
    return K.colsum(dy)


def _conv_wgrad(weight, x0, x1, dy, ks: int):
    cout = weight.shape[0]
    ctot = x0.shape[-1] + (0 if x1 is None else x1.shape[-1])
    kk = ks * ks
    return _wgrad_into_param(weight, x0, x1, dy, _sq_taps(ks), ctot * kk, kk, list(range(kk)))


class ConvFn(_Fn):

    @staticmethod
    def forward(ctx, x0, x1, weight, bias, residual, ksize: int, cache: PackCache):
        x0, x1, residual = _c(x0), _c(x1), _c(residual)
        cout = weight.shape[0]
        c0 = x0.shape[-1]
        c1 = 0 if x1 is None else x1.shape[-1]
        assert weight.numel() == cout * (c0 + c1) * ksize * ksize, (weight.shape, c0, c1, ksize)
        train = _train(ctx)
        wt = _conv_fwd_weight(cache, weight, cout, c0 + c1, ksize, train)
        ctx.wd = _conv_dgrad_weights(cache, weight, cout, c0, c1, ksize, train)
        y = K.igemm(x0, wt, a1=x1, taps=_sq_taps(ksize), bias=bias, residual=residual)
        ctx.save_for_backward(x0, x1, weight)
        ctx.ksize, ctx.has_bias, ctx.has_res = ksize, bias is not None, residual is not None
        return y

    @staticmethod
    def backward(ctx, dy):
        x0, x1, weight = ctx.saved_tensors
        dy = dy.contiguous()
        ntaps = [(-dh, -dw) for dh, dw in _sq_taps(ctx.ksize)]
        dx0 = dx1 = dwt = db = None
        if ctx.needs_input_grad[0]:
            dx0 = K.igemm(dy, ctx.wd[0], taps=ntaps)
        if x1 is not None and ctx.needs_input_grad[1]:
            dx1 = K.igemm(dy, ctx.wd[1], taps=ntaps)
        if ctx.needs_input_grad[2]:
            dwt = _conv_wgrad(weight, x0, x1, dy, ctx.ksize)
        if ctx.has_bias and ctx.needs_input_grad[3]:
            db = K.colsum(dy)
        dres = dy if (ctx.has_res and ctx.needs_input_grad[4]) else None
        return dx0, dx1, dwt, db, dres, None, None


class DownsampleFn(_Fn):

    TAPS = [(kh - 1, kw - 1) for kh in range(4) for kw in range(4)]

    @staticmethod
    def forward(ctx, x, weight, bias, cache: PackCache):
        x = x.contiguous()
        c = x.shape[-1]
        train = _train(ctx)
        wt = cache.get(weight, "fwd", (0, c, 16, c, c * 16, 16, list(range(16))), train)
        ctx.wd = {(ph, pw): cache.get(weight, ("dgrad", ph, pw), (0, c, 4, c, 16, c * 16, _phase(ph, pw)[1]), train)
                  for ph in (0, 1) for pw in (0, 1)} if train else None
        y = K.igemm(x, wt, taps=DownsampleFn.TAPS, stride=2, bias=bias)
        ctx.save_for_backward(x, weight)
        ctx.bias_ref = bias
        return y

    @staticmethod
    def backward(ctx, dy):
        x, weight = ctx.saved_tensors
        dy = dy.contiguous()
        n, h, w, c = x.shape
        dx = dwt = db = None
        if ctx.needs_input_grad[0]:
            dx = torch.empty_like(x)
            for (ph, pw), wd in ctx.wd.items():
                K.igemm(dy, wd, taps=_phase(ph, pw)[0], out=dx, out_hw=(h // 2, w // 2), out_place=(2, 2, ph, pw))
        if ctx.needs_input_grad[1]:
            dwt = _wgrad_into_param(weight, x, None, dy, DownsampleFn.TAPS, c * 16, 16, list(range(16)), stride=2)
        if ctx.needs_input_grad[2]:
            db = _bias_grad(ctx.bias_ref, dy)
        return dx, dwt, db, None


class UpsampleFn(_Fn):

    @staticmethod
    def forward(ctx, x, weight, bias, cache: PackCache):
        x = x.contiguous()
        n, h, w, c = x.shape
        out = torch.empty((n, 2 * h, 2 * w, c), dtype=H16, device=x.device)
        train = _train(ctx)
        ctx.wd = cache.get(weight, "dgrad", (0, c, 16, c, c * 16, 16, list(range(16))), train) if train else None
        for ph in (0, 1):
            for pw in (0, 1):
                taps, koff = _phase(ph, pw)
                wt = cache.get(weight, ("fwd", ph, pw), (0, c, 4, c, 16, c * 16, koff), train)
                K.igemm(x, wt, taps=taps, out=out, out_hw=(h, w), out_place=(2, 2, ph, pw), bias=bias)
        ctx.save_for_backward(x, weight)
        ctx.bias_ref = bias
        return out

    @staticmethod
    def backward(ctx, dy):
        x, weight = ctx.saved_tensors
        dy = dy.contiguous()
        n, h, w, c = x.shape
        dx = dwt = db = None
        if ctx.needs_input_grad[0]:
            dx = K.igemm(dy, ctx.wd, taps=DownsampleFn.TAPS, stride=2)
        if ctx.needs_input_grad[1]:
            into = None if _direct(weight) else torch.zeros_like(weight)
            for n_ph, (ph, pw) in enumerate([(0, 0), (0, 1), (1, 0), (1, 1)]):
                taps, koff = _phase(ph, pw)
                dwt = _wgrad_into_param(weight, x, None, dy, taps, 16, c * 16, koff, last=(n_ph == 3), into=into,
                                        grid_hw=(h, w), dy_place=(2, 2, ph, pw))
        if ctx.needs_input_grad[2]:
            db = _bias_grad(ctx.bias_ref, dy)
        return dx, dwt, db, None


class GroupNormSiLUFn(_Fn):

    @staticmethod
    def forward(ctx, x, gamma, beta, film, residual, B: int, G: int, eps: float):
        x, film, residual = x.contiguous(), _c(film), _c(residual)
        sums = K.gn_stats(x, B, G)
        out = K.gn_apply_fwd(x, sums, gamma, beta, film, residual, B, G, eps)
        ctx.save_for_backward(x, sums, gamma, beta, film)
        ctx.cfg = (B, G, eps, residual is not None)
        return out

    @staticmethod
    def backward(ctx, dout):
        x, sums, gamma, beta, film = ctx.saved_tensors
        B, G, eps, has_res = ctx.cfg
        dout = dout.contiguous()
        dx, dgamma, dbeta, dfilm = K.gn_bwd(x, dout, sums, gamma, beta, film, B, G, eps)
        return dx, dgamma, dbeta, dfilm, (dout if has_res else None), None, None, None


class LayerNormFn(_Fn):

    @staticmethod
    def forward(ctx, x, gamma, eps: float):
        x = x.contiguous()
        g = gamma.reshape(-1)
        ctx.save_for_backward(x, g)
        ctx.eps, ctx.gshape = eps, gamma.shape
        return K.ln_fwd(x, g, eps)

    @staticmethod
    def backward(ctx, dy):
        x, g = ctx.saved_tensors
        dx, dg = K.ln_bwd(x, g, dy.contiguous(), None, ctx.eps)
        return dx, dg.view(ctx.gshape), None


class TemporalAttnCoreFn(_Fn):

    @staticmethod
    def forward(ctx, qkv, pos_bias, cs, sn, B: int, F: int, HW: int, H: int, D: int):
        qkv, pos_bias = qkv.contiguous(), pos_bias.contiguous().float()
        scale = D ** -0.5
        out, lse = K.tattn_fwd(qkv, pos_bias, cs, sn, B, F, HW, H, D, scale)
        if F <= 4:
            ctx.save_for_backward(qkv, pos_bias, cs, sn)
        else:
            ctx.save_for_backward(qkv, pos_bias, cs, sn, out, lse)
        ctx.dims = (B, F, HW, H, D, scale)
        return out

    @staticmethod
    def backward(ctx, dout):
        B, F, HW, H, D, scale = ctx.dims
        if F <= 4:
            (qkv, pos_bias, cs, sn), out, lse = ctx.saved_tensors, None, None
        else:
            qkv, pos_bias, cs, sn, out, lse = ctx.saved_tensors
        dqkv, dbias = K.tattn_bwd(qkv, pos_bias, cs, sn, out, lse, dout.contiguous(), B, F, HW, H, D, scale)
        return dqkv, dbias, None, None, None, None, None, None, None


class MidAttnCoreFn(_Fn):

    @staticmethod
    def forward(ctx, qkv, NI: int, n: int, H: int, D: int):
        qkv = qkv.contiguous()
        out, lse = K.mattn_fwd(qkv, NI, n, H, D, D ** -0.5)
        ctx.save_for_backward(qkv, out, lse)
        ctx.dims = (NI, n, H, D)
        return out

    @staticmethod
    def backward(ctx, dout):
        qkv, out, lse = ctx.saved_tensors
        NI, n, H, D = ctx.dims
        return K.mattn_bwd(qkv, out, lse, dout.contiguous(), NI, n, H, D, D ** -0.5), None, None, None, None


class RelPosBiasFn(_Fn):

    @staticmethod
    def forward(ctx, weight, idx):
        ctx.save_for_backward(idx)
        ctx.shape = weight.shape
        return weight.detach()[idx].permute(2, 0, 1).float().contiguous()

    @staticmethod
    def backward(ctx, dbias):
        (idx,) = ctx.saved_tensors
        dw = torch.zeros(ctx.shape, dtype=dbias.dtype, device=dbias.device)
        dw.index_add_(0, idx.reshape(-1), dbias.permute(1, 2, 0).reshape(-1, ctx.shape[1]))
        return dw, None


class LinearAttnCoreFn(_Fn):

    @staticmethod
    def forward(ctx, qkv, NI: int, n: int, H: int, D: int):
        qkv = qkv.contiguous()
        scale = D ** -0.5
        out, ws = K.linattn_fwd(qkv, NI, n, H, D, scale)
        ctx.save_for_backward(qkv, ws)
        ctx.dims = (NI, n, H, D, scale)
        return out

    @staticmethod
    def backward(ctx, dout):
        qkv, ws = ctx.saved_tensors
        NI, n, H, D, scale = ctx.dims
        return K.linattn_bwd(qkv, ws, dout.contiguous(), NI, n, H, D, scale), None, None, None, None


class BlockMeta:

    def __init__(self, **kw):
        self.__dict__.update(kw)

    def __deepcopy__(self, memo):
        return BlockMeta(**{k: (PackCache() if isinstance(v, PackCache) else v) for k, v in self.__dict__.items()
                            if k != "fold_f1"})


class ResnetBlockFn(_Fn):

    @staticmethod
    def forward(ctx, x, x1, film, w1, b1, g1w, g1b, w2, b2, g2w, g2b, wres, bres, B, meta):
        x, x1, film = x.contiguous(), _c(x1), _c(film)
        G, eps = meta.G, meta.eps
        c0 = x.shape[-1]
        cx1 = 0 if x1 is None else x1.shape[-1]
        cout = w1.shape[0]
        train = _train(ctx)
        if wres is None:
            res = x
        else:
            res = K.igemm(x, _conv_fwd_weight(meta.cres, wres, cout, c0 + cx1, 1, train), a1=x1, bias=bres)
        F = x.shape[0] // B
        sums1 = K.zero_scratch((B, G, 2), x.device)
        y1 = K.igemm(x, _conv_fwd_weight(meta.c1, w1, cout, c0 + cx1, 3, train), a1=x1, taps=K.TAPS_3x3, bias=b1,
                     gn_sums=sums1, gn_frames=F)
        h1 = K.gn_apply_fwd(y1, sums1, g1w, g1b, film, None, B, G, eps)
        sums2 = K.zero_scratch((B, G, 2), x.device)
        y2 = K.igemm(h1, _conv_fwd_weight(meta.c2, w2, cout, cout, 3, train), taps=K.TAPS_3x3, bias=b2,
                     gn_sums=sums2, gn_frames=F)
        out = K.gn_apply_fwd(y2, sums2, g2w, g2b, None, res, B, G, eps)
        ctx.wd1 = _conv_dgrad_weights(meta.c1, w1, cout, c0, cx1, 3, train)
        ctx.wd2 = _conv_dgrad_weights(meta.c2, w2, cout, cout, 0, 3, train)
        ctx.wdres = None if wres is None else _conv_dgrad_weights(meta.cres, wres, cout, c0, cx1, 1, train)
        ctx.save_for_backward(x, x1, film, y1, sums1, h1, y2, sums2, w1, g1w, g1b, w2, g2w, g2b, wres, b1, b2, bres)
        ctx.cfg = (B, G, eps)
        return out

    @staticmethod
    def backward(ctx, dout):
        x, x1, film, y1, sums1, h1, y2, sums2, w1, g1w, g1b, w2, g2w, g2b, wres, b1, b2, bres = ctx.saved_tensors
        B, G, eps = ctx.cfg
        dout = dout.contiguous()
        ntaps = [(-dh, -dw) for dh, dw in K.TAPS_3x3]
        if _direct_all(g2w, g2b, b2):
            dy2, _, _, _, _ = K.gn_bwd(y2, dout, sums2, g2w, g2b, None, B, G, eps, conv_bias_grad=True,
                                       into=(g2w.grad, g2b.grad, b2.grad))
            _ready(g2w, g2b, b2)
            dg2w = dg2b = db2 = None
        else:
            dy2, dg2w, dg2b, _, db2 = K.gn_bwd(y2, dout, sums2, g2w, g2b, None, B, G, eps, conv_bias_grad=True)
        dw2 = _conv_wgrad(w2, h1, None, dy2, 3)
        dh1 = K.igemm(dy2, ctx.wd2[0], taps=ntaps)
        if _direct_all(g1w, g1b, b1):
            dy1, _, _, dfilm, _ = K.gn_bwd(y1, dh1, sums1, g1w, g1b, film, B, G, eps, conv_bias_grad=True,
                                           into=(g1w.grad, g1b.grad, b1.grad))
            _ready(g1w, g1b, b1)
            dg1w = dg1b = db1 = None
        else:
            dy1, dg1w, dg1b, dfilm, db1 = K.gn_bwd(y1, dh1, sums1, g1w, g1b, film, B, G, eps, conv_bias_grad=True)
        dw1 = _conv_wgrad(w1, x, x1, dy1, 3)
        dx = dx1 = dwres = dbres = None
        if wres is None:
            if ctx.needs_input_grad[0]:
                dx = K.igemm(dy1, ctx.wd1[0], taps=ntaps, residual=dout)
        else:
            if ctx.needs_input_grad[0]:
                r0 = K.igemm(dout, ctx.wdres[0])
                dx = K.igemm(dy1, ctx.wd1[0], taps=ntaps, residual=r0)
            if x1 is not None and ctx.needs_input_grad[1]:
                r1 = K.igemm(dout, ctx.wdres[1])
                dx1 = K.igemm(dy1, ctx.wd1[1], taps=ntaps, residual=r1)
            dwres = _conv_wgrad(wres, x, x1, dout, 1)
            if _direct_all(bres):
                with _on_side(dout):
                    K.colsum(dout, into=bres.grad)
                _ready(bres)
            else:
                dbres = K.colsum(dout)
        return dx, dx1, dfilm, dw1, db1, dg1w, dg1b, dw2, db2, dg2w, dg2b, dwres, dbres, None, None


def _qkv_backward(wqkv, wdq, xn, dqkv4):
    C, cout = xn.shape[-1], dqkv4.shape[-1]
    if C == 64 and cout % 128 == 0 and cout <= 768:
        if _direct(wqkv):
            dxn, _ = K.qkv_bwd(dqkv4, xn, wdq, dw_into=wqkv.grad)
            _ready(wqkv)
            return dxn, None
        dxn, dw = K.qkv_bwd(dqkv4, xn, wdq)
        return dxn, dw.view_as(wqkv)
    return K.igemm(dqkv4, wdq), _conv_wgrad(wqkv, xn, None, dqkv4, 1)


class TemporalAttnBlockFn(_Fn):

    @staticmethod
    def forward(ctx, x, gamma, wqkv, wout, pos_bias, cs, sn, B, F, meta):
        x = x.contiguous()
        NI, H_, W_, C = x.shape
        heads, D, eps = meta.heads, meta.dim_head, meta.eps
        hidden = heads * D
        g = gamma.reshape(-1)
        pos_bias = pos_bias.contiguous().float()
        train = _train(ctx)
        if F == 1 and not train and C == 64:
            wln, colsum = _fold_f1(meta, wqkv, wout, hidden, C, gamma=gamma)
            return K.igemm(x, wln, residual=x, ln_fold=(colsum, eps))
        xn = K.ln_fwd(x, g, eps)
        if F == 1 and not train:
            return K.igemm(xn, _fold_f1(meta, wqkv, wout, hidden, C), residual=x)
        wq = _conv_fwd_weight(meta.cq, wqkv, 3 * hidden, C, 1, train)
        if not train and K.tattn_proj_ok(C, F, H_ * W_, heads, D):
            o = K.tattn_proj_fwd(xn.view(-1, C), wq, pos_bias, cs, sn, B, F, H_ * W_, heads, D, D ** -0.5)
            return K.igemm(o.view(NI, H_, W_, hidden), _conv_fwd_weight(meta.co, wout, C, hidden, 1, train), residual=x)
        qkv = K.igemm(xn, wq)
        o, lse = K.tattn_fwd(qkv.view(-1, 3 * hidden), pos_bias, cs, sn, B, F, H_ * W_, heads, D, D ** -0.5)
        y = K.igemm(o.view(NI, H_, W_, hidden), _conv_fwd_weight(meta.co, wout, C, hidden, 1, train), residual=x)
        ctx.wdq = _conv_dgrad_weights(meta.cq, wqkv, 3 * hidden, C, 0, 1, train)[0]
        ctx.wdo = _conv_dgrad_weights(meta.co, wout, C, hidden, 0, 1, train)[0]
        saved = [x, g, xn, o, pos_bias, cs, sn, wqkv, wout, gamma, qkv]
        if F > 4:
            saved.append(lse)
        ctx.save_for_backward(*saved)
        ctx.cfg, ctx.gshape = (B, F, heads, D, eps), gamma.shape
        return y

    @staticmethod
    def backward(ctx, dy):
        saved = ctx.saved_tensors
        x, g, xn, o, pos_bias, cs, sn, wqkv, wout, gamma, qkv = saved[:11]
        lse = saved[11] if len(saved) > 11 else None
        B, F, heads, D, eps = ctx.cfg
        hidden = heads * D
        NI, H_, W_, C = x.shape
        dy = dy.contiguous()
        do = K.igemm(dy, ctx.wdo)
        dwout = _conv_wgrad(wout, o.view(NI, H_, W_, hidden), None, dy, 1)
        dqkv, dbias = K.tattn_bwd(qkv.view(-1, 3 * hidden), pos_bias, cs, sn, o if F > 4 else None, lse,
                                  do.view(-1, hidden), B, F, H_ * W_, heads, D, D ** -0.5)
        dqkv4 = dqkv.view(NI, H_, W_, 3 * hidden)
        dxn, dwqkv = _qkv_backward(wqkv, ctx.wdq, xn, dqkv4)
        if _direct_all(gamma):
            dx, _ = K.ln_bwd(x, g, dxn, dy, eps, into=gamma.grad.view(-1))
            _ready(gamma)
            dgamma = None
        else:
            dx, dg = K.ln_bwd(x, g, dxn, dy, eps)
            dgamma = dg.view(ctx.gshape)
        return dx, dgamma, dwqkv, dwout, dbias, None, None, None, None, None


class MidAttnBlockFn(_Fn):

    @staticmethod
    def forward(ctx, x, gamma, wqkv, wout, meta):
        x = x.contiguous()
        NI, H_, W_, C = x.shape
        heads, D, eps = meta.heads, meta.dim_head, meta.eps
        hidden, n = heads * D, H_ * W_
        g = gamma.reshape(-1)
        train = _train(ctx)
        xn = K.ln_fwd(x, g, eps)
        qkv = K.igemm(xn, _conv_fwd_weight(meta.cq, wqkv, 3 * hidden, C, 1, train))
        o, lse = K.mattn_fwd(qkv.view(-1, 3 * hidden), NI, n, heads, D, D ** -0.5)
        y = K.igemm(o.view(NI, H_, W_, hidden), _conv_fwd_weight(meta.co, wout, C, hidden, 1, train), residual=x)
        if train:
            ctx.wdq = _conv_dgrad_weights(meta.cq, wqkv, 3 * hidden, C, 0, 1, train)[0]
            ctx.wdo = _conv_dgrad_weights(meta.co, wout, C, hidden, 0, 1, train)[0]
            ctx.save_for_backward(x, g, xn, qkv, o, lse, wqkv, wout, gamma)
            ctx.cfg, ctx.gshape = (heads, D, eps), gamma.shape
        return y

    @staticmethod
    def backward(ctx, dy):
        x, g, xn, qkv, o, lse, wqkv, wout, gamma = ctx.saved_tensors
        heads, D, eps = ctx.cfg
        hidden = heads * D
        NI, H_, W_, C = x.shape
        dy = dy.contiguous()
        do = K.igemm(dy, ctx.wdo)
        dwout = _conv_wgrad(wout, o.view(NI, H_, W_, hidden), None, dy, 1)
        dqkv = K.mattn_bwd(qkv.view(-1, 3 * hidden), o.view(-1, hidden), lse, do.view(-1, hidden), NI, H_ * W_, heads, D,
                           D ** -0.5)
        dxn, dwqkv = _qkv_backward(wqkv, ctx.wdq, xn, dqkv.view(NI, H_, W_, 3 * hidden))
        if _direct_all(gamma):
            dx, _ = K.ln_bwd(x, g, dxn, dy, eps, into=gamma.grad.view(-1))
            _ready(gamma)
            dgamma = None
        else:
            dx, dg = K.ln_bwd(x, g, dxn, dy, eps)
            dgamma = dg.view(ctx.gshape)
        return dx, dgamma, dwqkv, dwout, None


class SpatialAttnBlockFn(_Fn):

    @staticmethod
    def forward(ctx, x, gamma, wqkv, wout, bout, meta):
        x = x.contiguous()
        NI, H_, W_, C = x.shape
        heads, D, eps = meta.heads, meta.dim_head, meta.eps
        hidden = heads * D
        g = gamma.reshape(-1)
        train = _train(ctx)
        xn = K.ln_fwd(x, g, eps)
        qkv = K.igemm(xn, _conv_fwd_weight(meta.cq, wqkv, 3 * hidden, C, 1, train))
        o, ws = K.linattn_fwd(qkv.view(-1, 3 * hidden), NI, H_ * W_, heads, D, D ** -0.5)
        y = K.igemm(o.view(NI, H_, W_, hidden), _conv_fwd_weight(meta.co, wout, C, hidden, 1, train), bias=bout,
                    residual=x)
        ctx.wdq = _conv_dgrad_weights(meta.cq, wqkv, 3 * hidden, C, 0, 1, train)[0]
        ctx.wdo = _conv_dgrad_weights(meta.co, wout, C, hidden, 0, 1, train)[0]
        ctx.save_for_backward(x, g, xn, qkv, o, ws, wqkv, wout, gamma, bout)
        ctx.cfg, ctx.gshape = (heads, D, eps), gamma.shape
        return y

    @staticmethod
    def backward(ctx, dy):
        x, g, xn, qkv, o, ws, wqkv, wout, gamma, bout = ctx.saved_tensors
        heads, D, eps = ctx.cfg
        hidden = heads * D
        NI, H_, W_, C = x.shape
        dy = dy.contiguous()
        do = K.igemm(dy, ctx.wdo)
        dwout = _conv_wgrad(wout, o.view(NI, H_, W_, hidden), None, dy, 1)
        if _direct_all(bout):
            with _on_side(dy):
                K.colsum(dy, into=bout.grad)
            _ready(bout)
            dbout = None
        else:
            dbout = K.colsum(dy)
        dqkv = K.linattn_bwd(qkv.view(-1, 3 * hidden), ws, do.view(-1, hidden), NI, H_ * W_, heads, D, D ** -0.5)
        dqkv4 = dqkv.view(NI, H_, W_, 3 * hidden)
        dxn, dwqkv = _qkv_backward(wqkv, ctx.wdq, xn, dqkv4)
        if _direct_all(gamma):
            dx, _ = K.ln_bwd(x, g, dxn, dy, eps, into=gamma.grad.view(-1))
            _ready(gamma)
            dgamma = None
        else:
            dx, dg = K.ln_bwd(x, g, dxn, dy, eps)
            dgamma = dg.view(ctx.gshape)
        return dx, dgamma, dwqkv, dwout, dbout, None


class InputConvFn(_Fn):

    @staticmethod
    def forward(ctx, x, cond, weight, bias, F: int):
        x, cond = x.contiguous().float(), cond.contiguous().float()
        B, H, W = x.shape[0], x.shape[-2], x.shape[-1]
        ks = weight.shape[-1]
        patches = K.input_patches(x, cond, B, F, H, W, ks)
        out = K.igemm(patches, K.input_weight_pack(weight.detach(), bias.detach()))
        if _train(ctx):
            ctx.save_for_backward(patches, weight, bias)
        return out

    @staticmethod
    def backward(ctx, dy):
        patches, weight, bias = ctx.saved_tensors
        nt = weight[0].numel()
        full = K.wgrad(patches, dy.contiguous())[:, 0, :]
        dw = (full[:, :nt] + full[:, nt:2 * nt]).view_as(weight)
        db = full[:, 2 * nt]
        if _direct_all(weight, bias):
            weight.grad.add_(dw)
            bias.grad.add_(db)
            _ready(weight, bias)
            return None, None, None, None, None
        return None, None, dw, db.contiguous(), None


class OutConvFn(_Fn):

    @staticmethod
    def forward(ctx, a, weight, bias, B: int, F: int, mid: int):
        a = a.contiguous()
        H, W = a.shape[1], a.shape[2]
        ctx.save_for_backward(a, weight)
        ctx.dims = (B, F, H, W, mid)
        return K.out_conv_fwd(a, weight, bias, B, F, H, W, mid)

    @staticmethod
    def backward(ctx, deps):
        a, weight = ctx.saved_tensors
        B, F, H, W, mid = ctx.dims
        da, dw, db = K.out_conv_bwd(a, weight, deps.contiguous().float(), B, F, H, W, mid)
        return da, dw, db, None, None, None


class SmallLinearFn(_Fn):

    @staticmethod
    def forward(ctx, x, weight, bias, act_in: bool):
        x = x.contiguous()
        ctx.save_for_backward(x, weight, bias)
        ctx.act_in = act_in
        return K.small_linear_fwd(x, weight, bias, act_in)

    @staticmethod
    def backward(ctx, dy):
        x, weight, bias = ctx.saved_tensors
        if _direct_all(weight, bias):
            dx, _, _ = K.small_linear_bwd(x, weight, dy.contiguous(), ctx.act_in, ctx.needs_input_grad[0],
                                          into=(weight.grad, bias.grad))
            _ready(weight, bias)
            return dx, None, None, None
        dx, dW, db = K.small_linear_bwd(x, weight, dy.contiguous(), ctx.act_in, ctx.needs_input_grad[0])
        return dx, dW, db, None


_FILM_TABLES: dict = {}


def _film_table(Ws, bs, direct: bool):
    key = (tuple(w.data_ptr() for w in Ws), tuple(b.data_ptr() for b in bs),
           tuple(w.grad.data_ptr() for w in Ws) + tuple(b.grad.data_ptr() for b in bs) if direct else None)
    tab = _FILM_TABLES.get(key)
    if tab is None:
        if len(_FILM_TABLES) > 16:
            _FILM_TABLES.clear()
        tab = K.film_table(Ws, bs, [w.grad for w in Ws], [b.grad for b in bs]) if direct else K.film_table(Ws, bs)
        _FILM_TABLES[key] = tab
    return tab


class FilmAllFn(_Fn):

    @staticmethod
    def forward(ctx, temb, *wb):
        x = temb.contiguous()
        Ws, bs = list(wb[0::2]), list(wb[1::2])
        Ns = [w.shape[0] for w in Ws]
        outs = K.film_fwd(x, _film_table(Ws, bs, False), Ns)
        ctx.save_for_backward(x, *wb)
        ctx.Ns = Ns
        return tuple(outs)

    @staticmethod
    def backward(ctx, *dys):
        x, wb = ctx.saved_tensors[0], ctx.saved_tensors[1:]
        Ws, bs = list(wb[0::2]), list(wb[1::2])
        B = x.shape[0]
        dy = torch.cat([(d if d is not None else x.new_zeros(B, n)).reshape(-1) for d, n in zip(dys, ctx.Ns)])
        if _direct_all(*Ws, *bs):
            dx = K.film_bwd(x, _film_table(Ws, bs, True), dy, ctx.Ns, ctx.needs_input_grad[0], accumulate=True)
            _ready(*Ws, *bs)
            return (dx,) + (None,) * len(wb)
        dWs, dbs = [torch.empty_like(w) for w in Ws], [torch.empty_like(b) for b in bs]
        dx = K.film_bwd(x, K.film_table(Ws, bs, dWs, dbs), dy, ctx.Ns, ctx.needs_input_grad[0], accumulate=False)
        grads = [None] * len(wb)
        grads[0::2], grads[1::2] = dWs, dbs
        return (dx,) + tuple(grads)


class MseLossFn(_Fn):

    @staticmethod
    def forward(ctx, eps, noise):
        loss, diff = K.mse_fwd(eps.contiguous(), noise.contiguous())
        ctx.save_for_backward(diff)
        return loss

    @staticmethod
    def backward(ctx, g):
        (diff,) = ctx.saved_tensors
        g = g.reshape(1).float().contiguous()
        return K.scale_by_scalar(diff, g, 2.0 / diff.numel()), None


def to_cl(x: torch.Tensor) -> Tuple[torch.Tensor, int, int]:
    B, C, F, H, W = x.shape
    return x.permute(0, 2, 3, 4, 1).reshape(B * F, H, W, C).to(H16).contiguous(), B, F


def from_cl(y: torch.Tensor, B: int, F: int) -> torch.Tensor:
    n, H, W, C = y.shape
    return y.view(B, F, H, W, C).permute(0, 4, 1, 2, 3)
```

### include/cesm_b200.h

```cpp
#ifndef CESM_B200_H
#define CESM_B200_H

#include <stddef.h>
#include <stdint.h>

#ifdef __cplusplus
extern "C" {
#endif

typedef enum cesm_status {
    CESM_OK = 0,
    CESM_ERR_INVALID = -1,
    CESM_ERR_CUDA = -2,
    CESM_ERR_INTERNAL = -3
} cesm_status;

const char* cesm_last_error(void);
const char* cesm_version(void);
long long cesm_launch_count(void);


#define CESM_MAX_TAPS 16

typedef struct cesm_igemm_args {
    const void* a0;
    const void* a1;
    int32_t c0, c1;
    int32_t n, h, w;
    int32_t stride;
    int32_t num_taps;
    int32_t tap_dh[CESM_MAX_TAPS];
    int32_t tap_dw[CESM_MAX_TAPS];
    const void* wt;
    int32_t cout;
    int32_t oh, ow;
    void* out;
    int32_t ldo;
    int32_t out_h, out_w, o_sh, o_sw, o_h0, o_w0;
    const float* bias;
    const void* residual;
    int32_t ldr;
    float* gn_sums;
    int32_t gn_groups;
    int32_t gn_frames;
    const float* ln_colsum;
    float ln_eps;
    int32_t reserved_;
} cesm_igemm_args;

int cesm_igemm(const cesm_igemm_args* args, void* stream);

typedef struct cesm_wgrad_args {
    const void* x0;
    const void* x1;
    int32_t c0, c1;
    int32_t n, h, w;
    int32_t stride;
    int32_t num_taps;
    int32_t tap_dh[CESM_MAX_TAPS];
    int32_t tap_dw[CESM_MAX_TAPS];
    const void* dy;
    int32_t cout;
    int32_t oh, ow;
    int32_t y_h, y_w, y_sh, y_sw, y_h0, y_w0;
    float* dw;
    long long dw_so, dw_si;
    int32_t dw_tap_off[CESM_MAX_TAPS];
} cesm_wgrad_args;

int cesm_wgrad(const cesm_wgrad_args* args, void* stream);

int cesm_pack_weight(const float* src, void* dst, int O, int T, int I, long long so, long long si,
                     const int32_t* tap_off, void* stream);
typedef struct cesm_pack_desc {
    const float* src;
    void* dst;
    int32_t O, T, I, pad_;
    long long so, si;
    int32_t tap_off[CESM_MAX_TAPS];
} cesm_pack_desc;
int cesm_pack_weights_batched(const cesm_pack_desc* descs_device, int n, void* stream);
int cesm_unpack_wgrads_batched(const cesm_pack_desc* descs_device, int n, void* stream);
int cesm_qkv_bwd(const void* dy, const void* x, const void* wt, void* dx, float* dw, long long dw_so, long long rows,
                 int cin, int cout, void* stream);

void cesm_set_prezeroed_scratch(int on);

#define CESM_OPT_STATE_FLOATS 16
int cesm_adamw_partials(void);
int cesm_adamw_step(float* p, const float* g, float* m, float* v, long long n, float* partials, float* state,
                    float beta1, float beta2, float eps, float max_norm, void* stream);
int cesm_adamw_ema_step(float* p, const float* g, float* m, float* v, float* ema, long long n, float* partials,
                        float* state, float beta1, float beta2, float eps, float max_norm, double ema_decay,
                        long long ema_start, void* stream);
int cesm_unpack_wgrad(const float* src, float* dst, int O, int T, int I, long long so, long long si,
                      const int32_t* tap_off, int accumulate, void* stream);
int cesm_colsum(const void* x, float* out, long long M, int C, int accumulate, void* stream);

int cesm_gn_stats(const void* x, float* sums, int B, long long P, int C, int G, void* stream);
int cesm_gn_apply_fwd(const void* x, const float* sums, const float* gamma, const float* beta, const float* film,
                      const void* residual, void* out, int B, long long P, int C, int G, float eps, void* stream);
int cesm_gn_bwd(const void* x, const void* dout, const float* sums, const float* gamma, const float* beta,
                const float* film, float* csum, void* dx, float* dgamma, float* dbeta, float* dfilm,
                float* dconv_bias, int B, long long P, int C, int G, float eps, int accumulate_params, void* stream);

int cesm_ln_fwd(const void* x, const float* gamma, void* out, long long M, int C, float eps, void* stream);
int cesm_ln_bwd(const void* x, const float* gamma, const void* dy, const void* dres, void* dx, float* dgamma,
                long long M, int C, float eps, int accumulate, void* stream);

int cesm_tattn_fwd(const void* qkv, const float* bias, const float* cs, const float* sn, void* out, float* lse,
                   int B, int F, int HW, int H, int dim_head, float scale, void* stream);
int cesm_tattn_bwd(const void* qkv, const float* bias, const float* cs, const float* sn, const void* out,
                   const float* lse, const void* dout, void* dqkv, float* dbias, int B, int F, int HW, int H,
                   int dim_head, float scale, void* stream);

int cesm_tattn_proj_fwd(const void* xn, const void* wqkv, const float* bias, const float* cs, const float* sn, void* out,
                        int B, int F, int HW, int H, int dim_head, int cin, float scale, void* stream);

int cesm_tattn_long_max_frames(void);
int cesm_tattn_long_fwd(const void* qkv, const float* bias_diag, const float* cs, const float* sn, void* out,
                        float* lse, int B, int F, int HW, int H, int dim_head, float scale, void* stream);
int cesm_tattn_long_bwd(const void* qkv, const float* bias_diag, const float* cs, const float* sn, const void* out,
                        const float* lse, const void* dout, void* dqkv, float* dbias_diag, int B, int F, int HW, int H,
                        int dim_head, float scale, void* stream);

int cesm_mattn_fwd(const void* qkv, void* out, float* lse, int NI, int n, int H, int dim_head, float scale, void* stream);
int cesm_mattn_bwd(const void* qkv, const void* out, const float* lse, const void* dout, void* dqkv, float* delta, int NI,
                   int n, int H, int dim_head, float scale, void* stream);

size_t cesm_linattn_ws_floats(int NI, int H);
int cesm_linattn_fwd(const void* qkv, float* ws, void* out, int NI, int n, int H, int dim_head, float scale,
                     void* stream);
int cesm_linattn_bwd(const void* qkv, float* ws, const void* dout, float* scratch, void* dqkv, int NI, int n, int H,
                     int dim_head, float scale, void* stream);

typedef struct cesm_film_desc {
    const float* W;
    const float* bias;
    float* dW;
    float* db;
    int32_t N, n0;
} cesm_film_desc;
int cesm_film_fwd(const float* x, const cesm_film_desc* layers_device, float* y, int n_layers, int n_total, int B,
                  int K, void* stream);
int cesm_film_bwd(const float* x, const cesm_film_desc* layers_device, const float* dy, int n_layers, int n_total,
                  float* dx, int B, int K, int accumulate, void* stream);

int cesm_gather_windows(const float* cond, const float* tgt, const int* plan, float* cond_out, float* x0_out, int B,
                        int T, int M, int H, int W, int K, int h, int w, void* stream);

int cesm_input_patches(const float* in0, const float* in1, int f0, int f1, void* out, int B, int F, int H, int W,
                       int ks, int kpad, void* stream);
int cesm_input_weight_pack(const float* w, const float* bias, void* out, int cout, int ks, int kpad, void* stream);
int cesm_input_conv_fwd(const float* in0, const float* in1, int f0, int f1, const float* w, const float* bias,
                        void* out, int B, int F, int H, int W, int ks, int cout, void* stream);
int cesm_input_conv_wgrad(const float* in0, const float* in1, int f0, int f1, const void* dy, float* dw, float* db,
                          int B, int F, int H, int W, int ks, int cout, void* stream);
int cesm_out_conv_fwd(const void* a, const float* w, const float* bias, float* eps, int B, int F, int mid,
                      long long HW, int C, void* stream);
int cesm_out_conv_bwd(const void* a, const float* w, const float* deps, void* da, float* dw, float* db, int B, int F,
                      int mid, long long HW, int C, void* stream);

int cesm_sinusoidal(const long long* t, float* out, int B, int dim, void* stream);
int cesm_small_linear_fwd(const float* x, const float* W, const float* bias, float* y, int B, int K, int N,
                          int act_silu_in, void* stream);
int cesm_small_linear_bwd(const float* x, const float* W, const float* dy, float* dx, float* dW, float* db, int B,
                          int K, int N, int act_silu_in, int accumulate, void* stream);

int cesm_q_sample(const float* x0, const float* noise, const long long* t, const float* sqrt_ac,
                  const float* sqrt_1mac, float* xt, int B, long long per_sample, void* stream);
int cesm_mse_fwd(const float* eps, const float* noise, float* diff, float* loss, long long total, void* stream);
int cesm_scale_by_scalar(const float* in, const float* gscale, float factor, float* out, long long total,
                         void* stream);
int cesm_p_sample(const float* xt, const float* eps, const float* z, const long long* t, const float* betas,
                  const float* sqrt_1mac, const float* sqrt_recip_a, const float* post_var, float* out, int B,
                  long long per_sample, void* stream);
int cesm_ddim_step(const float* xt, const float* eps, const float* z, const long long* t, const float* coef,
                   const long long* next_t, long long* t_out, float* out, int T, int B, long long per_sample,
                   void* stream);
int cesm_dpm_step(const float* xt, const float* eps, float* hist, const long long* t, const float* coef,
                  const long long* next_t, long long* t_out, float* out, int T, int B, long long per_sample,
                  void* stream);

#ifdef __cplusplus
}
#endif
#endif
```

Before: 188.7.

## Fuse linear-attention backward with QKV projection backward in a tcgen05 kernel

Adds a persistent kernel that computes dq/dk/dv rows of the linear-attention backward in registers, stages them in shared memory, and feeds them directly into the QKV projection's dgrad and wgrad GEMMs using TMA, mbarriers and tensor memory. The goal is to avoid writing the dqkv tensor to global memory and reading it back, and to remove the separate GEMM launches. The old per-row math is moved into a shared header so both paths use it. The fused path only runs for C=64, 8 heads of 32, and n a multiple of 128; other shapes fall back to the old path. It adds complex pipeline synchronisation and a weight-gradient accumulation that could limit parallelism.

```diff
diff --git a/cesm_emulator_b200/_lib.py b/cesm_emulator_b200/_lib.py
--- a/cesm_emulator_b200/_lib.py
+++ b/cesm_emulator_b200/_lib.py
@@ -119,6 +119,7 @@
     "cesm_mattn_bwd": [_P, _P, _P, _P, _P, _P, _I, _I, _I, _I, _F, _P],
     "cesm_linattn_fwd": [_P, _P, _P, _I, _I, _I, _I, _F, _P],
     "cesm_linattn_bwd": [_P, _P, _P, _P, _P, _I, _I, _I, _I, _F, _P],
+    "cesm_linattn_qkv_bwd": [_P, _P, _P, _P, _P, _P, _P, _P, _L, _I, _I, _I, _I, _F, _P],
     "cesm_film_fwd": [_P, _P, _P, _I, _I, _I, _I, _P],
     "cesm_film_bwd": [_P, _P, _P, _I, _I, _P, _I, _I, _I, _P],
     "cesm_gather_windows": [_P, _P, _P, _P, _P, _I, _I, _I, _I, _I, _I, _I, _I, _P],
diff --git a/cesm_emulator_b200/csrc/linattn.cu b/cesm_emulator_b200/csrc/linattn.cu
--- a/cesm_emulator_b200/csrc/linattn.cu
+++ b/cesm_emulator_b200/csrc/linattn.cu
@@ -1,9 +1,8 @@
 #include "api_common.h"
-#include "common.cuh"
+#include "linattn_common.cuh"
 
 namespace cesm {
 
-static constexpr int LD = 32;
 static constexpr int SPITCH = 40;
 
 __device__ __forceinline__ void ldmatrix_x4_trans(uint32_t (&r)[4], uint32_t addr) {
@@ -11,38 +10,6 @@
                  : "=r"(r[0]), "=r"(r[1]), "=r"(r[2]), "=r"(r[3])
                  : "r"(addr));
 }
-__device__ __forceinline__ void mma_16816(float (&c)[4], const uint32_t (&a)[4], uint32_t b0, uint32_t b1) {
-    asm volatile(
-        "mma.sync.aligned.m16n8k16.row.col.f32.f16.f16.f32 {%0, %1, %2, %3}, {%4, %5, %6, %7}, {%8, %9}, "
-        "{%0, %1, %2, %3};"
-        : "+f"(c[0]), "+f"(c[1]), "+f"(c[2]), "+f"(c[3])
-        : "r"(a[0]), "r"(a[1]), "r"(a[2]), "r"(a[3]), "r"(b0), "r"(b1));
-}
-__device__ __forceinline__ uint32_t enc_ordered(float f) {
-    const uint32_t b = __float_as_uint(f);
-    return (b & 0x80000000u) ? ~b : (b | 0x80000000u);
-}
-__device__ __forceinline__ float dec_ordered(uint32_t u) {
-    return __uint_as_float((u & 0x80000000u) ? (u & 0x7fffffffu) : ~u);
-}
-__device__ __forceinline__ void unpack8(const uint4& u, float (&f)[8]) {
-    float2 a = unpack_h2(u.x), b = unpack_h2(u.y), c = unpack_h2(u.z), d = unpack_h2(u.w);
-    f[0] = a.x; f[1] = a.y; f[2] = b.x; f[3] = b.y; f[4] = c.x; f[5] = c.y; f[6] = d.x; f[7] = d.y;
-}
-__device__ __forceinline__ uint4 pack8(const float (&f)[8]) {
-    uint4 u;
-    u.x = pack_h2(f[0], f[1]); u.y = pack_h2(f[2], f[3]);
-    u.z = pack_h2(f[4], f[5]); u.w = pack_h2(f[6], f[7]);
-    return u;
-}
-__device__ __forceinline__ float quad_max(float v) {
-    v = fmaxf(v, __shfl_xor_sync(0xffffffffu, v, 1));
-    return fmaxf(v, __shfl_xor_sync(0xffffffffu, v, 2));
-}
-__device__ __forceinline__ float quad_sum(float v) {
-    v += __shfl_xor_sync(0xffffffffu, v, 1);
-    return v + __shfl_xor_sync(0xffffffffu, v, 2);
-}
 
 __device__ __forceinline__ void cp_async16(uint32_t dst, const void* src) {
     asm volatile("cp.async.cg.shared.global [%0], [%1], 16;" ::"r"(dst), "l"(src) : "memory");
@@ -53,16 +20,6 @@
     asm volatile("cp.async.wait_group %0;" ::"n"(N) : "memory");
 }
 static constexpr int kTileBytes = 16 * SPITCH * 2;
-
-struct LaWs {
-    uint32_t* kmax;
-    float* z;
-    float* ctx;
-};
-__device__ __forceinline__ LaWs la_ws(float* ws, int ni, int HD, int H) {
-    float* base = ws + (size_t)ni * (2 * HD + (size_t)H * LD * LD);
-    return {reinterpret_cast<uint32_t*>(base), base + HD, base + 2 * HD};
-}
 
 __global__ void __launch_bounds__(256)
 la_colmax_kernel(const h16* __restrict__ qkv, float* __restrict__ ws, int n, int H, int rows_per_block) {
@@ -280,58 +237,6 @@
 #pragma unroll
     for (int e = 0; e < LD; ++e) s = fmaf(W.ctx[hd * LD + e], dc[e], s);
     delta[idx] = s;
-}
-
-__device__ __forceinline__ int phi32(int L) { return ((L >> 1) & 3) * 8 + (L >> 3) * 2 + (L & 1); }
-
-template <bool TRANS>
-__device__ __forceinline__ void load_bfrag32(const float* __restrict__ M, int g, int t, uint32_t (&b)[2][4][2]) {
-#pragma unroll
-    for (int ks = 0; ks < 2; ++ks)
-#pragma unroll
-        for (int j = 0; j < 4; ++j) {
-            const int nn = phi32(8 * j + g);
-#pragma unroll
-            for (int hi = 0; hi < 2; ++hi) {
-                const int k0 = phi32(16 * ks + 8 * hi + 2 * t), k1 = k0 + 1;
-                b[ks][j][hi] = TRANS ? pack_h2(M[nn * LD + k0], M[nn * LD + k1])
-                                     : pack_h2(M[k0 * LD + nn], M[k1 * LD + nn]);
-            }
-        }
-}
-__device__ __forceinline__ void rows_to_afrag(const uint4& lo, const uint4& hi, uint32_t (&a)[2][4]) {
-    a[0][0] = lo.x; a[0][1] = hi.x; a[0][2] = lo.y; a[0][3] = hi.y;
-    a[1][0] = lo.z; a[1][1] = hi.z; a[1][2] = lo.w; a[1][3] = hi.w;
-}
-__device__ __forceinline__ void frag_gemm(const uint32_t (&a)[2][4], const uint32_t (&b)[2][4][2], float (&c)[4][4]) {
-#pragma unroll
-    for (int j = 0; j < 4; ++j) {
-        c[j][0] = c[j][1] = c[j][2] = c[j][3] = 0.f;
-#pragma unroll
-        for (int ks = 0; ks < 2; ++ks) mma_16816(c[j], a[ks], b[ks][j][0], b[ks][j][1]);
-    }
-}
-__device__ __forceinline__ void c_to_rows(const float (&c)[4][4], float (&o)[2][8]) {
-#pragma unroll
-    for (int j = 0; j < 4; ++j) {
-        o[0][2 * j] = c[j][0]; o[0][2 * j + 1] = c[j][1];
-        o[1][2 * j] = c[j][2]; o[1][2 * j + 1] = c[j][3];
-    }
-}
-__device__ __forceinline__ void row_softmax(float (&f)[8]) {
-    float m = f[0];
-#pragma unroll
-    for (int i = 1; i < 8; ++i) m = fmaxf(m, f[i]);
-    m = quad_max(m) * kLog2e;
-    float s = 0.f;
-#pragma unroll
-    for (int i = 0; i < 8; ++i) {
-        f[i] = exp_sub(f[i], m);
-        s += f[i];
-    }
-    const float inv = 1.f / quad_sum(s);
-#pragma unroll
-    for (int i = 0; i < 8; ++i) f[i] *= inv;
 }
 
 static constexpr int APPLY_MT = 2;
@@ -472,63 +377,35 @@
             issue_loads(p + (RING_STAGES - 1) * 16, ns);
         }
         cp_async_wait<RING_STAGES - 1>();
-        float sm[2][8];
-        uint4 ud[2], uv[2], uk[2];
+        uint4 ud[2], uq[2], uk[2], uv[2];
 #pragma unroll
         for (int h2 = 0; h2 < 2; ++h2) {
             const uint32_t st = ring + stage * kStage + h2 * 4 * kVec;
             ud[h2] = lds16(st);
-            unpack8(lds16(st + kVec), sm[h2]);
+            uq[h2] = lds16(st + kVec);
             uk[h2] = lds16(st + 2 * kVec);
             uv[h2] = lds16(st + 3 * kVec);
         }
         if (++stage == RING_STAGES) stage = 0;
-#pragma unroll
-        for (int h2 = 0; h2 < 2; ++h2) row_softmax(sm[h2]);
-        uint32_t a[2][4];
-        float cfr[4][4], o[2][8];
-        rows_to_afrag(ud[0], ud[1], a);
-        frag_gemm(a, b_ctxT, cfr);
-        c_to_rows(cfr, o);
-#pragma unroll
-        for (int h2 = 0; h2 < 2; ++h2) {
-            float dot = 0.f;
-#pragma unroll
-            for (int i = 0; i < 8; ++i) dot = fmaf(sm[h2][i], o[h2][i], dot);
-            dot = quad_sum(dot);
-#pragma unroll
-            for (int i = 0; i < 8; ++i) o[h2][i] = sm[h2][i] * scale * (o[h2][i] - dot);
-            const int row = p + r + 8 * h2;
-            if (row < p1) *reinterpret_cast<uint4*>(gbase + (size_t)row * ld) = pack8(o[h2]);
-        }
-        rows_to_afrag(uv[0], uv[1], a);
-        frag_gemm(a, b_dctxT, cfr);
-        c_to_rows(cfr, o);
-        uint4 ukh[2];
-#pragma unroll
-        for (int h2 = 0; h2 < 2; ++h2) {
-            float kh[8], km[8], dl[8];
-            unpack8(uk[h2], kh);
-            *reinterpret_cast<float4*>(km) = *reinterpret_cast<const float4*>(kml);
-            *reinterpret_cast<float4*>(km + 4) = *reinterpret_cast<const float4*>(kml + 4);
-            *reinterpret_cast<float4*>(dl) = *reinterpret_cast<const float4*>(del);
-            *reinterpret_cast<float4*>(dl + 4) = *reinterpret_cast<const float4*>(del + 4);
-#pragma unroll
-            for (int i = 0; i < 8; ++i) {
-                kh[i] = exp_sub(kh[i], km[i]);
-                o[h2][i] = kh[i] * (o[h2][i] - dl[i]);
-            }
-            ukh[h2] = pack8(kh);
-            const int row = p + r + 8 * h2;
-            if (row < p1) *reinterpret_cast<uint4*>(gbase + (size_t)row * ld + HD) = pack8(o[h2]);
-        }
-        rows_to_afrag(ukh[0], ukh[1], a);
-        frag_gemm(a, b_dctx, cfr);
-        c_to_rows(cfr, o);
+        uint4 dq[2], dk[2], dv[2];
+        la_bwd_dq_rows(uq, ud, b_ctxT, scale, dq);
 #pragma unroll
         for (int h2 = 0; h2 < 2; ++h2) {
             const int row = p + r + 8 * h2;
-            if (row < p1) *reinterpret_cast<uint4*>(gbase + (size_t)row * ld + 2 * HD) = pack8(o[h2]);
+            if (row < p1) *reinterpret_cast<uint4*>(gbase + (size_t)row * ld) = dq[h2];
+        }
+        uint4 ukh[2];
+        la_bwd_dk_rows(uk, uv, kml, del, b_dctxT, dk, ukh);
+#pragma unroll
+        for (int h2 = 0; h2 < 2; ++h2) {
+            const int row = p + r + 8 * h2;
+            if (row < p1) *reinterpret_cast<uint4*>(gbase + (size_t)row * ld + HD) = dk[h2];
+        }
+        la_bwd_dv_rows(ukh, b_dctx, dv);
+#pragma unroll
+        for (int h2 = 0; h2 < 2; ++h2) {
+            const int row = p + r + 8 * h2;
+            if (row < p1) *reinterpret_cast<uint4*>(gbase + (size_t)row * ld + 2 * HD) = dv[h2];
         }
     }
 }
@@ -579,8 +456,8 @@
     return CESM_OK;
 }
 
-extern "C" int cesm_linattn_bwd(const void* qkv, float* ws, const void* dout, float* scratch, void* dqkv, int NI, int n,
-                                int H, int dim_head, float scale, void* stream) {
+extern "C" int cesm_linattn_bwd_ctx(const void* qkv, float* ws, const void* dout, float* scratch, int NI, int n, int H,
+                                    int dim_head, float scale, void* stream) {
     CESM_REQUIRE(dim_head == LD, "linear attention kernel needs dim_head == 32 (got %d)", dim_head);
     CESM_REQUIRE(H >= 1 && H <= 8, "linear attention kernel supports 1..8 heads (got %d)", H);
     cudaStream_t st = as_stream(stream);
@@ -595,6 +472,18 @@
     CESM_CHECK_LAUNCH();
     launch_pdl(la_delta_kernel, ceil_div(NI * H * LD, 128), 128, 0, st, ws, dctx, delta, H, NI);
     CESM_CHECK_LAUNCH();
+    return CESM_OK;
+}
+
+extern "C" int cesm_linattn_bwd(const void* qkv, float* ws, const void* dout, float* scratch, void* dqkv, int NI, int n,
+                                int H, int dim_head, float scale, void* stream) {
+    const int rc = cesm_linattn_bwd_ctx(qkv, ws, dout, scratch, NI, n, H, dim_head, scale, stream);
+    if (rc) return rc;
+    cudaStream_t st = as_stream(stream);
+    float* dctx = scratch;
+    float* delta = scratch + (size_t)NI * H * LD * LD;
+    const int chunk = la_chunk(n, NI);
+    dim3 grid(ceil_div(n, chunk), NI);
     const size_t sh_bwd = (size_t)RING_STAGES * 8 * 256 * 16;
     static bool bwd_cfg = false;
     if (!bwd_cfg) {
diff --git a/cesm_emulator_b200/csrc/linattn_common.cuh b/cesm_emulator_b200/csrc/linattn_common.cuh
--- /dev/null
+++ b/cesm_emulator_b200/csrc/linattn_common.cuh
@@ -0,0 +1,162 @@
+#pragma once
+#include "common.cuh"
+
+namespace cesm {
+
+static constexpr int LD = 32;
+
+__device__ __forceinline__ void mma_16816(float (&c)[4], const uint32_t (&a)[4], uint32_t b0, uint32_t b1) {
+    asm volatile(
+        "mma.sync.aligned.m16n8k16.row.col.f32.f16.f16.f32 {%0, %1, %2, %3}, {%4, %5, %6, %7}, {%8, %9}, "
+        "{%0, %1, %2, %3};"
+        : "+f"(c[0]), "+f"(c[1]), "+f"(c[2]), "+f"(c[3])
+        : "r"(a[0]), "r"(a[1]), "r"(a[2]), "r"(a[3]), "r"(b0), "r"(b1));
+}
+__device__ __forceinline__ uint32_t enc_ordered(float f) {
+    const uint32_t b = __float_as_uint(f);
+    return (b & 0x80000000u) ? ~b : (b | 0x80000000u);
+}
+__device__ __forceinline__ float dec_ordered(uint32_t u) {
+    return __uint_as_float((u & 0x80000000u) ? (u & 0x7fffffffu) : ~u);
+}
+__device__ __forceinline__ void unpack8(const uint4& u, float (&f)[8]) {
+    float2 a = unpack_h2(u.x), b = unpack_h2(u.y), c = unpack_h2(u.z), d = unpack_h2(u.w);
+    f[0] = a.x; f[1] = a.y; f[2] = b.x; f[3] = b.y; f[4] = c.x; f[5] = c.y; f[6] = d.x; f[7] = d.y;
+}
+__device__ __forceinline__ uint4 pack8(const float (&f)[8]) {
+    uint4 u;
+    u.x = pack_h2(f[0], f[1]); u.y = pack_h2(f[2], f[3]);
+    u.z = pack_h2(f[4], f[5]); u.w = pack_h2(f[6], f[7]);
+    return u;
+}
+__device__ __forceinline__ float quad_max(float v) {
+    v = fmaxf(v, __shfl_xor_sync(0xffffffffu, v, 1));
+    return fmaxf(v, __shfl_xor_sync(0xffffffffu, v, 2));
+}
+__device__ __forceinline__ float quad_sum(float v) {
+    v += __shfl_xor_sync(0xffffffffu, v, 1);
+    return v + __shfl_xor_sync(0xffffffffu, v, 2);
+}
+
+struct LaWs {
+    uint32_t* kmax;
+    float* z;
+    float* ctx;
+};
+__device__ __forceinline__ LaWs la_ws(float* ws, int ni, int HD, int H) {
+    float* base = ws + (size_t)ni * (2 * HD + (size_t)H * LD * LD);
+    return {reinterpret_cast<uint32_t*>(base), base + HD, base + 2 * HD};
+}
+
+__device__ __forceinline__ int phi32(int L) { return ((L >> 1) & 3) * 8 + (L >> 3) * 2 + (L & 1); }
+
+template <bool TRANS>
+__device__ __forceinline__ void load_bfrag32(const float* __restrict__ M, int g, int t, uint32_t (&b)[2][4][2]) {
+#pragma unroll
+    for (int ks = 0; ks < 2; ++ks)
+#pragma unroll
+        for (int j = 0; j < 4; ++j) {
+            const int nn = phi32(8 * j + g);
+#pragma unroll
+            for (int hi = 0; hi < 2; ++hi) {
+                const int k0 = phi32(16 * ks + 8 * hi + 2 * t), k1 = k0 + 1;
+                b[ks][j][hi] = TRANS ? pack_h2(M[nn * LD + k0], M[nn * LD + k1])
+                                     : pack_h2(M[k0 * LD + nn], M[k1 * LD + nn]);
+            }
+        }
+}
+__device__ __forceinline__ void rows_to_afrag(const uint4& lo, const uint4& hi, uint32_t (&a)[2][4]) {
+    a[0][0] = lo.x; a[0][1] = hi.x; a[0][2] = lo.y; a[0][3] = hi.y;
+    a[1][0] = lo.z; a[1][1] = hi.z; a[1][2] = lo.w; a[1][3] = hi.w;
+}
+__device__ __forceinline__ void frag_gemm(const uint32_t (&a)[2][4], const uint32_t (&b)[2][4][2], float (&c)[4][4]) {
+#pragma unroll
+    for (int j = 0; j < 4; ++j) {
+        c[j][0] = c[j][1] = c[j][2] = c[j][3] = 0.f;
+#pragma unroll
+        for (int ks = 0; ks < 2; ++ks) mma_16816(c[j], a[ks], b[ks][j][0], b[ks][j][1]);
+    }
+}
+__device__ __forceinline__ void c_to_rows(const float (&c)[4][4], float (&o)[2][8]) {
+#pragma unroll
+    for (int j = 0; j < 4; ++j) {
+        o[0][2 * j] = c[j][0]; o[0][2 * j + 1] = c[j][1];
+        o[1][2 * j] = c[j][2]; o[1][2 * j + 1] = c[j][3];
+    }
+}
+__device__ __forceinline__ void row_softmax(float (&f)[8]) {
+    float m = f[0];
+#pragma unroll
+    for (int i = 1; i < 8; ++i) m = fmaxf(m, f[i]);
+    m = quad_max(m) * kLog2e;
+    float s = 0.f;
+#pragma unroll
+    for (int i = 0; i < 8; ++i) {
+        f[i] = exp_sub(f[i], m);
+        s += f[i];
+    }
+    const float inv = 1.f / quad_sum(s);
+#pragma unroll
+    for (int i = 0; i < 8; ++i) f[i] *= inv;
+}
+
+__device__ __forceinline__ void la_bwd_dq_rows(const uint4 (&uq)[2], const uint4 (&ud)[2],
+                                               const uint32_t (&b_ctxT)[2][4][2], float scale, uint4 (&dq)[2]) {
+    float sm[2][8];
+#pragma unroll
+    for (int h2 = 0; h2 < 2; ++h2) {
+        unpack8(uq[h2], sm[h2]);
+        row_softmax(sm[h2]);
+    }
+    uint32_t a[2][4];
+    float cfr[4][4], o[2][8];
+    rows_to_afrag(ud[0], ud[1], a);
+    frag_gemm(a, b_ctxT, cfr);
+    c_to_rows(cfr, o);
+#pragma unroll
+    for (int h2 = 0; h2 < 2; ++h2) {
+        float dot = 0.f;
+#pragma unroll
+        for (int i = 0; i < 8; ++i) dot = fmaf(sm[h2][i], o[h2][i], dot);
+        dot = quad_sum(dot);
+#pragma unroll
+        for (int i = 0; i < 8; ++i) o[h2][i] = sm[h2][i] * scale * (o[h2][i] - dot);
+        dq[h2] = pack8(o[h2]);
+    }
+}
+__device__ __forceinline__ void la_bwd_dk_rows(const uint4 (&uk)[2], const uint4 (&uv)[2], const float* kml,
+                                               const float* del, const uint32_t (&b_dctxT)[2][4][2], uint4 (&dk)[2],
+                                               uint4 (&ukh)[2]) {
+    uint32_t a[2][4];
+    float cfr[4][4], o[2][8];
+    rows_to_afrag(uv[0], uv[1], a);
+    frag_gemm(a, b_dctxT, cfr);
+    c_to_rows(cfr, o);
+#pragma unroll
+    for (int h2 = 0; h2 < 2; ++h2) {
+        float kh[8], km[8], dl[8];
+        unpack8(uk[h2], kh);
+        *reinterpret_cast<float4*>(km) = *reinterpret_cast<const float4*>(kml);
+        *reinterpret_cast<float4*>(km + 4) = *reinterpret_cast<const float4*>(kml + 4);
+        *reinterpret_cast<float4*>(dl) = *reinterpret_cast<const float4*>(del);
+        *reinterpret_cast<float4*>(dl + 4) = *reinterpret_cast<const float4*>(del + 4);
+#pragma unroll
+        for (int i = 0; i < 8; ++i) {
+            kh[i] = exp_sub(kh[i], km[i]);
+            o[h2][i] = kh[i] * (o[h2][i] - dl[i]);
+        }
+        ukh[h2] = pack8(kh);
+        dk[h2] = pack8(o[h2]);
+    }
+}
+__device__ __forceinline__ void la_bwd_dv_rows(const uint4 (&ukh)[2], const uint32_t (&b_dctx)[2][4][2], uint4 (&dv)[2]) {
+    uint32_t a[2][4];
+    float cfr[4][4], o[2][8];
+    rows_to_afrag(ukh[0], ukh[1], a);
+    frag_gemm(a, b_dctx, cfr);
+    c_to_rows(cfr, o);
+    dv[0] = pack8(o[0]);
+    dv[1] = pack8(o[1]);
+}
+
+}
diff --git a/cesm_emulator_b200/csrc/linattn_qkvbwd.cu b/cesm_emulator_b200/csrc/linattn_qkvbwd.cu
--- /dev/null
+++ b/cesm_emulator_b200/csrc/linattn_qkvbwd.cu
@@ -0,0 +1,403 @@
+#include "api_common.h"
+#include "linattn_common.cuh"
+
+namespace cesm {
+
+static constexpr int LQ_C = 64;
+static constexpr int LQ_H = 8;
+static constexpr int LQ_HD = LQ_H * LD;
+static constexpr int LQ_COUT = 3 * LQ_HD;
+static constexpr int LQ_TILE = 128;
+static constexpr int LQ_CHUNKS = LQ_COUT / 128;
+static constexpr int LQ_SUB = LQ_TILE * 128;
+static constexpr int LQ_CHUNK = 2 * LQ_SUB;
+static constexpr int LQ_WSUB = LQ_C * 128;
+static constexpr int LQ_WCHUNK = 2 * LQ_WSUB;
+static constexpr int LQ_STAGES = 4;
+static constexpr int LQ_WSTAGES = 2;
+static constexpr int LQ_XSTAGES = 2;
+static constexpr int LQ_TAB = 8 * 2 * LD * 4;
+static constexpr int LQ_SMEM =
+    1024 + LQ_STAGES * LQ_CHUNK + LQ_WSTAGES * LQ_WCHUNK + LQ_XSTAGES * LQ_SUB + LQ_TAB + 256;
+static constexpr int LQ_THREADS = 512;
+
+struct LqMaps {
+    CUtensorMap x;
+    CUtensorMap w;
+};
+struct LqParams {
+    const h16* qkv;
+    const h16* dout;
+    float* ws;
+    const float* dctx;
+    const float* delta;
+    h16* dx;
+    float* dw;
+    long long so;
+    int n, tiles;
+    float scale;
+};
+
+__device__ __forceinline__ void sts16(uint32_t addr, const uint4& u) {
+    asm volatile("st.shared.v4.b32 [%0], {%1, %2, %3, %4};" ::"r"(addr), "r"(u.x), "r"(u.y), "r"(u.z), "r"(u.w)
+                 : "memory");
+}
+
+__device__ __forceinline__ void l2_prefetch_bulk(const void* p, uint32_t bytes) {
+    asm volatile("cp.async.bulk.prefetch.L2.global [%0], %1;" ::"l"(p), "r"(bytes) : "memory");
+}
+
+__global__ void __launch_bounds__(LQ_THREADS, 1)
+linattn_qkv_bwd_kernel(const __grid_constant__ LqMaps maps, const LqParams p) {
+    pdl_trigger();
+    extern __shared__ uint8_t smem_raw[];
+    const uint32_t smem_base = (smem_u32(smem_raw) + 1023u) & ~1023u;
+    uint8_t* smem_gen = smem_raw + (smem_base - smem_u32(smem_raw));
+    const uint32_t w_base = smem_base + LQ_STAGES * LQ_CHUNK;
+    const uint32_t x_base = w_base + LQ_WSTAGES * LQ_WCHUNK;
+    const uint32_t tab_base = x_base + LQ_XSTAGES * LQ_SUB;
+    const uint32_t bar_base = tab_base + LQ_TAB;
+    auto s_full = [&](int s) { return bar_base + 8u * s; };
+    auto s_empty = [&](int s) { return bar_base + 8u * (4 + s); };
+    auto w_full = [&](int s) { return bar_base + 8u * (8 + s); };
+    auto w_empty = [&](int s) { return bar_base + 8u * (10 + s); };
+    auto x_full = [&](int s) { return bar_base + 8u * (12 + s); };
+    auto x_empty = [&](int s) { return bar_base + 8u * (14 + s); };
+    auto d1_full = [&](int s) { return bar_base + 8u * (16 + s); };
+    auto d1_empty = [&](int s) { return bar_base + 8u * (18 + s); };
+    const uint32_t d2_full = bar_base + 8u * 20;
+    const uint32_t tmem_ptr_addr = bar_base + 8u * 21;
+    volatile uint32_t* tmem_ptr_gen = reinterpret_cast<volatile uint32_t*>(smem_gen + (tmem_ptr_addr - smem_base));
+
+    const int warp = threadIdx.x >> 5, lane = threadIdx.x & 31;
+    const int tile_begin = (int)((long long)blockIdx.x * p.tiles / gridDim.x);
+    const int tile_end = (int)((long long)(blockIdx.x + 1) * p.tiles / gridDim.x);
+    if (threadIdx.x == 0) {
+        tma_prefetch_desc(&maps.x);
+        tma_prefetch_desc(&maps.w);
+        for (int s = 0; s < LQ_STAGES; ++s) {
+            mbar_init(s_full(s), 128);
+            mbar_init(s_empty(s), 1);
+        }
+        for (int s = 0; s < 2; ++s) {
+            mbar_init(w_full(s), 1);
+            mbar_init(w_empty(s), 1);
+            mbar_init(x_full(s), 1);
+            mbar_init(x_empty(s), 1);
+            mbar_init(d1_full(s), 1);
+            mbar_init(d1_empty(s), 4);
+        }
+        mbar_init(d2_full, 1);
+        fence_barrier_init();
+    }
+    if (warp == 2) tmem_alloc(tmem_ptr_addr, 512);
+    tc_fence_before();
+    __syncthreads();
+    tc_fence_after();
+    const uint32_t tmem_base = *tmem_ptr_gen;
+    const uint32_t tmem_d1 = tmem_base;
+    const uint32_t tmem_d2 = tmem_base + 128;
+    if (warp == 0 && lane == 0) {
+        pdl_wait();
+        int xs = 0, wsl = 0;
+        uint32_t xph = 0, wph = 0;
+        for (int tile = tile_begin; tile < tile_end; ++tile) {
+            mbar_wait(x_empty(xs), xph ^ 1u, 51);
+            mbar_arrive_expect_tx(x_full(xs), LQ_SUB);
+            tma_load_2d(x_base + xs * LQ_SUB, &maps.x, x_full(xs), 0, tile * LQ_TILE);
+            if (++xs == LQ_XSTAGES) {
+                xs = 0;
+                xph ^= 1u;
+            }
+            for (int c = 0; c < LQ_CHUNKS; ++c) {
+                mbar_wait(w_empty(wsl), wph ^ 1u, 52);
+                const uint32_t wb = w_base + wsl * LQ_WCHUNK;
+                mbar_arrive_expect_tx(w_full(wsl), LQ_WCHUNK);
+                tma_load_2d(wb, &maps.w, w_full(wsl), c * 128, 0);
+                tma_load_2d(wb + LQ_WSUB, &maps.w, w_full(wsl), c * 128 + 64, 0);
+                if (++wsl == LQ_WSTAGES) {
+                    wsl = 0;
+                    wph ^= 1u;
+                }
+            }
+        }
+    } else if (warp == 1) {
+        constexpr uint32_t idesc_dg = make_idesc_f16(LQ_TILE, LQ_C, 0, 0);
+        constexpr uint32_t idesc_wg = make_idesc_f16(128, LQ_C, 1, 1);
+        if (elect_one()) {
+            const uint64_t dk = make_smem_desc_sw128(0, 0, 1024);
+            const uint64_t dmn = make_smem_desc_sw128(0, LQ_SUB, 1024);
+            int xs = 0, wsl = 0, acc = 0, it = 0, kc = 0;
+            uint32_t xph = 0, wph = 0, accph = 0;
+            for (int tile = tile_begin; tile < tile_end; ++tile, ++it) {
+                mbar_wait(d1_empty(acc), accph ^ 1u, 53);
+                mbar_wait(x_full(xs), xph, 54);
+                tc_fence_after();
+                const uint32_t x16 = (x_base + xs * LQ_SUB) >> 4;
+                const uint32_t d1 = tmem_d1 + acc * 64;
+                for (int c = 0; c < LQ_CHUNKS; ++c, ++kc) {
+                    const int st = kc & (LQ_STAGES - 1);
+                    mbar_wait(s_full(st), (uint32_t)(kc / LQ_STAGES) & 1u, 55);
+                    mbar_wait(w_full(wsl), wph, 56);
+                    tc_fence_after();
+                    const uint32_t a16 = (smem_base + st * LQ_CHUNK) >> 4;
+                    const uint32_t w16 = (w_base + wsl * LQ_WCHUNK) >> 4;
+#pragma unroll
+                    for (int k = 0; k < 8; ++k) {
+                        const uint32_t ao = a16 + (k >> 2) * (LQ_SUB >> 4) + (k & 3) * 2;
+                        const uint32_t bo = w16 + (k >> 2) * (LQ_WSUB >> 4) + (k & 3) * 2;
+                        umma_f16(d1, dk | (uint64_t)ao, dk | (uint64_t)bo, idesc_dg, k == 0 ? (uint32_t)(c != 0) : 1u);
+                    }
+                    const uint32_t d2 = tmem_d2 + c * 64;
+#pragma unroll
+                    for (int k = 0; k < 8; ++k)
+                        umma_f16(d2, dmn | (uint64_t)(a16 + k * 128), dmn | (uint64_t)(x16 + k * 128), idesc_wg,
+                                 k == 0 ? (uint32_t)(it != 0) : 1u);
+                    umma_commit(s_empty(st));
+                    umma_commit(w_empty(wsl));
+                    if (++wsl == LQ_WSTAGES) {
+                        wsl = 0;
+                        wph ^= 1u;
+                    }
+                }
+                umma_commit(x_empty(xs));
+                umma_commit(d1_full(acc));
+                if (++xs == LQ_XSTAGES) {
+                    xs = 0;
+                    xph ^= 1u;
+                }
+                if (++acc == 2) {
+                    acc = 0;
+                    accph ^= 1u;
+                }
+            }
+            umma_commit(d2_full);
+        }
+        __syncwarp();
+    } else if (warp >= 4 && warp < 8) {
+        const int q = warp & 3;
+        const uint32_t lane_base = static_cast<uint32_t>(q * 32) << 16;
+        int acc = 0;
+        uint32_t accph = 0;
+        for (int tile = tile_begin; tile < tile_end; ++tile) {
+            mbar_wait(d1_full(acc), accph, 57);
+            tc_fence_after();
+            const long long row = (long long)tile * LQ_TILE + q * 32 + lane;
+#pragma unroll
+            for (int half = 0; half < 2; ++half) {
+                uint32_t v[32];
+                tmem_ld_32x32(tmem_d1 + acc * 64 + half * 32 + lane_base, v);
+                tmem_ld_wait();
+                uint4* dst = reinterpret_cast<uint4*>(p.dx + row * LQ_C + half * 32);
+#pragma unroll
+                for (int j = 0; j < 4; ++j) {
+                    uint4 u;
+                    u.x = pack_h2(__uint_as_float(v[8 * j + 0]), __uint_as_float(v[8 * j + 1]));
+                    u.y = pack_h2(__uint_as_float(v[8 * j + 2]), __uint_as_float(v[8 * j + 3]));
+                    u.z = pack_h2(__uint_as_float(v[8 * j + 4]), __uint_as_float(v[8 * j + 5]));
+                    u.w = pack_h2(__uint_as_float(v[8 * j + 6]), __uint_as_float(v[8 * j + 7]));
+                    dst[j] = u;
+                }
+            }
+            tc_fence_before();
+            __syncwarp();
+            if (lane == 0) mbar_arrive(d1_empty(acc));
+            if (++acc == 2) {
+                acc = 0;
+                accph ^= 1u;
+            }
+        }
+        if (tile_begin < tile_end) {
+            mbar_wait(d2_full, 0, 58);
+            tc_fence_after();
+            float* tr = reinterpret_cast<float*>(smem_gen) + q * (32 * 33);
+            for (int c = 0; c < LQ_CHUNKS; ++c) {
+                float* base = p.dw + (long long)(c * 128 + q * 32) * p.so;
+#pragma unroll 1
+                for (int half = 0; half < 2; ++half) {
+                    uint32_t v[32];
+                    tmem_ld_32x32(tmem_d2 + c * 64 + half * 32 + lane_base, v);
+                    tmem_ld_wait();
+                    __syncwarp();
+#pragma unroll
+                    for (int i = 0; i < 32; ++i) tr[lane * 33 + i] = __uint_as_float(v[i]);
+                    __syncwarp();
+#pragma unroll 8
+                    for (int co = 0; co < 32; ++co) atomicAdd(base + (long long)co * p.so + half * 32 + lane, tr[co * 33 + lane]);
+                }
+            }
+        }
+    } else if (warp >= 8) {
+        const int mw = warp - 8, G = mw >> 2, hw = mw & 3, h = 4 * G + hw;
+        const int g = lane >> 2, t = lane & 3;
+        const int pr = ((g & 1) << 2) | (g >> 1);
+        const uint32_t col_sub = (hw >> 1) * LQ_SUB;
+        const uint32_t col16 = (uint32_t)(((hw & 1) << 2) | t);
+        float* tab = reinterpret_cast<float*>(smem_gen + (tab_base - smem_base)) + mw * 2 * LD;
+        auto st_off = [&](int px) { return col_sub + px * 128u + ((col16 ^ (uint32_t)(px & 7)) << 4); };
+        uint32_t b_dctxT[2][4][2], b_dctx[2][4][2];
+        const float* ctx = nullptr;
+        int cur_ni = -1;
+        const bool prefetcher = lane == 0 && hw == 0;
+        auto prefetch_tile = [&](int tl) {
+            const long long r = (long long)tl * LQ_TILE;
+            if (G == 0) {
+                const uint8_t* b = reinterpret_cast<const uint8_t*>(p.qkv + r * LQ_COUT);
+                for (int i = 0; i < LQ_TILE * LQ_COUT * 2; i += 32768) l2_prefetch_bulk(b + i, 32768u);
+            } else {
+                const uint8_t* b = reinterpret_cast<const uint8_t*>(p.dout + r * LQ_HD);
+                for (int i = 0; i < LQ_TILE * LQ_HD * 2; i += 32768) l2_prefetch_bulk(b + i, 32768u);
+            }
+        };
+        pdl_wait();
+        if (prefetcher && tile_begin < tile_end) prefetch_tile(tile_begin);
+        int it = 0;
+        for (int tile = tile_begin; tile < tile_end; ++tile, ++it) {
+            const long long row0 = (long long)tile * LQ_TILE;
+            if (prefetcher && tile + 1 < tile_end) prefetch_tile(tile + 1);
+            const int ni = (int)(row0 / p.n);
+            if (ni != cur_ni) {
+                cur_ni = ni;
+                const LaWs W = la_ws(p.ws, ni, LQ_HD, LQ_H);
+                const float* dcx = p.dctx + ((size_t)ni * LQ_H + h) * LD * LD;
+                ctx = W.ctx + (size_t)h * LD * LD;
+                load_bfrag32<true>(dcx, g, t, b_dctxT);
+                load_bfrag32<false>(dcx, g, t, b_dctx);
+                __syncwarp();
+                tab[lane] = (dec_ordered(W.kmax[h * LD + lane]) + __logf(W.z[h * LD + lane])) * kLog2e;
+                tab[LD + lane] = p.delta[(size_t)ni * LQ_HD + h * LD + lane];
+                __syncwarp();
+            }
+            const h16* qrow = p.qkv + row0 * LQ_COUT + h * LD + t * 8;
+            const h16* drow = p.dout + row0 * LQ_HD + h * LD + t * 8;
+            auto ld2 = [&](const h16* base, long long stride, int s, uint4 (&u)[2]) {
+                u[0] = __ldg(reinterpret_cast<const uint4*>(base + (16 * s + pr) * stride));
+                u[1] = __ldg(reinterpret_cast<const uint4*>(base + (16 * s + pr + 8) * stride));
+            };
+            {
+                const int kc = 6 * it + G, st = kc & (LQ_STAGES - 1);
+                const uint32_t sb = smem_base + st * LQ_CHUNK;
+                uint4 uq[2], ud[2];
+                ld2(qrow, LQ_COUT, 0, uq);
+                ld2(drow, LQ_HD, 0, ud);
+                uint32_t b_ctxT[2][4][2];
+                load_bfrag32<true>(ctx, g, t, b_ctxT);
+                mbar_wait(s_empty(st), ((uint32_t)(kc / LQ_STAGES) & 1u) ^ 1u, 59);
+#pragma unroll 1
+                for (int s = 0; s < LQ_TILE / 16; ++s) {
+                    uint4 nq[2], nd[2];
+                    if (s + 1 < LQ_TILE / 16) {
+                        ld2(qrow, LQ_COUT, s + 1, nq);
+                        ld2(drow, LQ_HD, s + 1, nd);
+                    }
+                    uint4 dq[2];
+                    la_bwd_dq_rows(uq, ud, b_ctxT, p.scale, dq);
+#pragma unroll
+                    for (int h2 = 0; h2 < 2; ++h2) sts16(sb + st_off(16 * s + pr + 8 * h2), dq[h2]);
+#pragma unroll
+                    for (int h2 = 0; h2 < 2; ++h2) {
+                        uq[h2] = nq[h2];
+                        ud[h2] = nd[h2];
+                    }
+                }
+                fence_proxy_async();
+                mbar_arrive(s_full(st));
+            }
+            {
+                const int kk = 6 * it + 2 + G, kv = kk + 2;
+                const int sk = kk & (LQ_STAGES - 1), sv = kv & (LQ_STAGES - 1);
+                const uint32_t bk = smem_base + sk * LQ_CHUNK, bv = smem_base + sv * LQ_CHUNK;
+                uint4 uk[2], uv[2];
+                ld2(qrow + LQ_HD, LQ_COUT, 0, uk);
+                ld2(qrow + 2 * LQ_HD, LQ_COUT, 0, uv);
+                mbar_wait(s_empty(sk), ((uint32_t)(kk / LQ_STAGES) & 1u) ^ 1u, 60);
+                mbar_wait(s_empty(sv), ((uint32_t)(kv / LQ_STAGES) & 1u) ^ 1u, 61);
+                const float* kml = tab + t * 8;
+                const float* del = tab + LD + t * 8;
+#pragma unroll 1
+                for (int s = 0; s < LQ_TILE / 16; ++s) {
+                    uint4 nk[2], nv[2];
+                    if (s + 1 < LQ_TILE / 16) {
+                        ld2(qrow + LQ_HD, LQ_COUT, s + 1, nk);
+                        ld2(qrow + 2 * LQ_HD, LQ_COUT, s + 1, nv);
+                    }
+                    uint4 dk[2], dv[2], ukh[2];
+                    la_bwd_dk_rows(uk, uv, kml, del, b_dctxT, dk, ukh);
+#pragma unroll
+                    for (int h2 = 0; h2 < 2; ++h2) sts16(bk + st_off(16 * s + pr + 8 * h2), dk[h2]);
+                    la_bwd_dv_rows(ukh, b_dctx, dv);
+#pragma unroll
+                    for (int h2 = 0; h2 < 2; ++h2) sts16(bv + st_off(16 * s + pr + 8 * h2), dv[h2]);
+#pragma unroll
+                    for (int h2 = 0; h2 < 2; ++h2) {
+                        uk[h2] = nk[h2];
+                        uv[h2] = nv[h2];
+                    }
+                }
+                fence_proxy_async();
+                mbar_arrive(s_full(sk));
+                mbar_arrive(s_full(sv));
+            }
+        }
+    }
+    tc_fence_before();
+    __syncthreads();
+    if (warp == 2) tmem_dealloc(tmem_base, 512);
+}
+
+}
+
+using namespace cesm;
+
+extern "C" int cesm_linattn_bwd_ctx(const void* qkv, float* ws, const void* dout, float* scratch, int NI, int n, int H,
+                                    int dim_head, float scale, void* stream);
+
+extern "C" int cesm_linattn_qkv_bwd(const void* qkv, float* ws, const void* dout, float* scratch, const void* xn,
+                                    const void* wt, void* dx, float* dw, long long dw_so, int NI, int n, int H,
+                                    int dim_head, float scale, void* stream) {
+    CESM_REQUIRE(H == LQ_H && dim_head == LD, "linattn_qkv_bwd is specialised for 8 heads of 32 (got %d x %d)", H,
+                 dim_head);
+    CESM_REQUIRE(NI > 0 && n > 0 && n % LQ_TILE == 0, "linattn_qkv_bwd needs n a multiple of %d (n=%d)", LQ_TILE, n);
+    CESM_REQUIRE(dw_so >= LQ_C, "bad dw stride");
+    const int rc = cesm_linattn_bwd_ctx(qkv, ws, dout, scratch, NI, n, H, dim_head, scale, stream);
+    if (rc) return rc;
+    const long long rows = (long long)NI * n;
+    LqMaps maps;
+    {
+        const uint64_t dims[2] = {(uint64_t)LQ_C, (uint64_t)rows};
+        const uint64_t str[1] = {(uint64_t)LQ_C * 2};
+        const uint32_t box[2] = {64u, (uint32_t)LQ_TILE};
+        int e = get_tensor_map_h16(&maps.x, xn, 2, dims, str, box);
+        if (e) return e;
+    }
+    {
+        const uint64_t dims[2] = {(uint64_t)LQ_COUT, (uint64_t)LQ_C};
+        const uint64_t str[1] = {(uint64_t)LQ_COUT * 2};
+        const uint32_t box[2] = {64u, (uint32_t)LQ_C};
+        int e = get_tensor_map_h16(&maps.w, wt, 2, dims, str, box);
+        if (e) return e;
+    }
+    LqParams p;
+    p.qkv = (const h16*)qkv;
+    p.dout = (const h16*)dout;
+    p.ws = ws;
+    p.dctx = scratch;
+    p.delta = scratch + (size_t)NI * H * LD * LD;
+    p.dx = (h16*)dx;
+    p.dw = dw;
+    p.so = dw_so;
+    p.n = n;
+    p.tiles = (int)(rows / LQ_TILE);
+    p.scale = scale;
+    static bool cfg = false;
+    if (!cfg) {
+        CESM_CHECK_CUDA(cudaFuncSetAttribute(linattn_qkv_bwd_kernel, cudaFuncAttributeMaxDynamicSharedMemorySize, LQ_SMEM));
+        cfg = true;
+    }
+    int sms = 148, dev = 0;
+    if (cudaGetDevice(&dev) == cudaSuccess) cudaDeviceGetAttribute(&sms, cudaDevAttrMultiProcessorCount, dev);
+    const int grid = p.tiles < sms ? p.tiles : sms;
+    launch_pdl(linattn_qkv_bwd_kernel, grid, LQ_THREADS, LQ_SMEM, as_stream(stream), maps, p);
+    CESM_CHECK_LAUNCH();
+    return CESM_OK;
+}
diff --git a/cesm_emulator_b200/kernels.py b/cesm_emulator_b200/kernels.py
--- a/cesm_emulator_b200/kernels.py
+++ b/cesm_emulator_b200/kernels.py
@@ -420,6 +420,30 @@
     return dqkv
 
 
+def linattn_qkv_bwd(qkv, ws, dout, xn, wt, NI: int, n: int, H: int, D: int, scale: float,
+                    dw_into: Optional[torch.Tensor] = None):
+    _req_cuda(qkv, ws, dout, xn, wt, dw_into)
+    assert qkv.dtype == H16 and dout.dtype == H16 and xn.dtype == H16 and wt.dtype == H16
+    cout, cin = 3 * H * D, xn.shape[-1]
+    rows = NI * n
+    assert qkv.numel() == rows * cout and dout.numel() == rows * H * D and xn.numel() == rows * cin
+    assert tuple(wt.shape) == (cin, cout)
+    scratch = zero_scratch((NI * H * D * D + NI * H * D,), qkv.device)
+    dx = torch.empty_like(xn)
+    if dw_into is None:
+        dw = torch.zeros((cout, cin), dtype=torch.float32, device=xn.device)
+    else:
+        assert dw_into.dtype == torch.float32 and dw_into.numel() == cout * cin
+        dw = dw_into
+    meta = None
+    if _lib.PROFILER is not None:
+        meta = {"kind": "la_qkv", "flops": 4.0 * rows * cout * cin,
+                "bytes": 2.0 * rows * (cout + H * D + 2 * cin) + 4.0 * (ws.numel() + scratch.numel())}
+    _lib.call("cesm_linattn_qkv_bwd", _ptr(qkv), _ptr(ws), _ptr(dout), _ptr(scratch), _ptr(xn), _ptr(wt), _ptr(dx),
+              _ptr(dw), cin, NI, n, H, D, scale, _stream(), _meta=meta)
+    return dx, dw
+
+
 def gather_windows(cond, tgt, plan, cond_out, x0_out) -> None:
     _req_cuda(cond, tgt, plan, cond_out, x0_out)
     assert cond.dtype == tgt.dtype == cond_out.dtype == x0_out.dtype == torch.float32 and plan.dtype == torch.int32
diff --git a/cesm_emulator_b200/ops.py b/cesm_emulator_b200/ops.py
--- a/cesm_emulator_b200/ops.py
+++ b/cesm_emulator_b200/ops.py
@@ -732,9 +732,19 @@
             dbout = None
         else:
             dbout = K.colsum(dy)
-        dqkv = K.linattn_bwd(qkv.view(-1, 3 * hidden), ws, do.view(-1, hidden), NI, H_ * W_, heads, D, D ** -0.5)
-        dqkv4 = dqkv.view(NI, H_, W_, 3 * hidden)
-        dxn, dwqkv = _qkv_backward(wqkv, ctx.wdq, xn, dqkv4)
+        n = H_ * W_
+        if C == 64 and heads == 8 and D == 32 and n % 128 == 0:
+            direct = _direct(wqkv)
+            dxn, dw = K.linattn_qkv_bwd(qkv.view(-1, 3 * hidden), ws, do.view(-1, hidden), xn, ctx.wdq, NI, n,
+                                        heads, D, D ** -0.5, dw_into=wqkv.grad if direct else None)
+            if direct:
+                _ready(wqkv)
+                dwqkv = None
+            else:
+                dwqkv = dw.view_as(wqkv)
+        else:
+            dqkv = K.linattn_bwd(qkv.view(-1, 3 * hidden), ws, do.view(-1, hidden), NI, n, heads, D, D ** -0.5)
+            dxn, dwqkv = _qkv_backward(wqkv, ctx.wdq, xn, dqkv.view(NI, H_, W_, 3 * hidden))
         if _direct_all(gamma):
             dx, _ = K.ln_bwd(x, g, dxn, dy, eps, into=gamma.grad.view(-1))
             _ready(gamma)
diff --git a/include/cesm_b200.h b/include/cesm_b200.h
--- a/include/cesm_b200.h
+++ b/include/cesm_b200.h
@@ -133,6 +133,9 @@
                      void* stream);
 int cesm_linattn_bwd(const void* qkv, float* ws, const void* dout, float* scratch, void* dqkv, int NI, int n, int H,
                      int dim_head, float scale, void* stream);
+int cesm_linattn_qkv_bwd(const void* qkv, float* ws, const void* dout, float* scratch, const void* xn, const void* wt,
+                         void* dx, float* dw, long long dw_so, int NI, int n, int H, int dim_head, float scale,
+                         void* stream);
 
 typedef struct cesm_film_desc {
     const float* W;
```

New measurement: 186.7 (median of 6 runs). 0.99x the previous value.
